# mataiyuan/ASD-SLAM

Measured on AMD Instinct MI355X. Metric: frames/sec end-to-end tracking+LocalBA, KITTI 00 mono @2000 keypoints, higher is better.
Workload: dtype f32

## Files before the change

asd-slam_amd/csrc/asdnet.hip:

```cpp
#include "ctx.h"

#include <algorithm>
#include <cmath>
#include <cstring>

typedef float f32x16 __attribute__((ext_vector_type(16)));
typedef float f32x4 __attribute__((ext_vector_type(4)));


namespace {

struct LayerSpec { int cout, cin, k, stride, pad; };
const LayerSpec kLayers[7] = {{32, 1, 3, 1, 1},   {32, 32, 3, 1, 1},   {64, 32, 3, 2, 1},  {64, 64, 3, 1, 1},
                              {128, 64, 3, 2, 1}, {128, 128, 3, 1, 1}, {128, 128, 8, 1, 0}};

template <int CIN, int COUT, int HIN, int S, int ROWS, int WM, int WN, int KC, int PP = 1, int RING = 2>
struct ConvCfg {
  static constexpr int HO = HIN / S;
  static constexpr int INROWS = (ROWS - 1) * S + 3;
  static constexpr int INCOLS = (HO - 1) * S + 3;
  static constexpr int CPAD = CIN + 4;
  static constexpr int NW = WM * WN;
  static constexpr int NTH = 64 * NW;
  static constexpr int M_PATCH = ROWS * HO;
  static constexpr int M_WG = PP * M_PATCH;
  static constexpr int MT = M_WG / 32 / WM;
  static constexpr int NT = COUT / 32 / WN;
  static constexpr int NCC = CIN / KC;
  static constexpr int NSTAGE = 9 * NCC;
  static constexpr int WCHUNK = KC * COUT;
  static constexpr int WQUADS = WCHUNK / 4;
  static constexpr int WREGS = (WQUADS + NTH - 1) / NTH;
  static constexpr int ACT_FLOATS = INROWS * INCOLS * CPAD;
  static constexpr int LDS_BYTES = (PP * ACT_FLOATS + RING * WCHUNK) * 4;
  static_assert(RING == 2 || RING == 3, "weight ring depth");
  static_assert(NW == 4 || NW == 8, "4 or 8 waves per workgroup");
  static_assert(M_WG % (32 * WM) == 0 && COUT % (32 * WN) == 0, "tile split");
  static_assert(WQUADS % NTH == 0 || WQUADS < NTH, "weight stage: whole float4 rounds per thread, or a single partial round");
  static_assert(HO % ROWS == 0 && CIN % KC == 0 && KC % 8 == 0, "shape");
  static_assert(PP == 1 || ROWS == HO, "several patches per workgroup only for whole-patch bands");
  static_assert(M_PATCH % 32 == 0, "32-pixel MFMA tiles must not straddle patches");
};

template <int CIN, int COUT, int HIN, int S, int ROWS, int WM, int WN, int KC, int PP = 1, int RING = 2, int ABL = 0, bool FUSE1 = false>
__global__ __launch_bounds__(64 * WM * WN) void k_conv_mfma(const void* __restrict__ in_, const float* __restrict__ wimg,
                                                           const float* __restrict__ bias, float* __restrict__ out,
                                                           const float* __restrict__ w1, const float* __restrict__ b1, int n) {
  using C = ConvCfg<CIN, COUT, HIN, S, ROWS, WM, WN, KC, PP, RING>;
  constexpr int NTH = C::NTH;
  extern __shared__ __attribute__((aligned(16))) float smem[];
  float* sact = smem;
  float* sw = smem + PP * C::ACT_FLOATS;
  const int t = threadIdx.x, lane = t & 63, wave = t >> 6;
  const int wm = wave / WN, wn = wave % WN;
  constexpr int BANDS = C::HO / ROWS;
  const int patch = (blockIdx.x / BANDS) * PP, band = blockIdx.x % BANDS;
  const int r0 = band * ROWS;

  if constexpr (FUSE1) {
    static_assert(!FUSE1 || (CIN == 32 && HIN == 32 && S == 1 && PP == 1), "conv1 fusion is for conv2 only");
    float* pin = sw + RING * C::WCHUNK;
    float* wsh = pin + (ROWS + 4) * 36;
    float* red = wsh + 320;
    const uint8_t* patches = static_cast<const uint8_t*>(in_);
    for (int i = t; i < (ROWS + 4) * 36; i += NTH) pin[i] = 0.f;
    for (int i = t; i < 288; i += NTH) wsh[i] = w1[i];
    if (t < 32) wsh[288 + t] = b1[t];
    const bool ld = C::NW == 4 || wave < 4;
    const uchar4 v = ld ? reinterpret_cast<const uchar4*>(patches + (size_t)patch * 1024)[t] : make_uchar4(0, 0, 0, 0);
    const float inv255 = (float)(1.0 / 255);
    float x[4] = {v.x * inv255, v.y * inv255, v.z * inv255, v.w * inv255};
#pragma unroll
    for (int k = 0; k < 4; ++k) asm volatile("" : "+v"(x[k]));
    float s = (x[0] + x[1]) + (x[2] + x[3]);
    for (int off = 32; off >= 1; off >>= 1) s += __shfl_xor(s, off);
    if (lane == 0 && ld) red[wave] = s;
    asd_syncthreads();
    const float mean = ((red[0] + red[1]) + (red[2] + red[3])) * (1.0f / 1024.0f);
    float d[4], ss = 0.f;
    for (int k = 0; k < 4; ++k) { d[k] = x[k] - mean; ss += d[k] * d[k]; }
    for (int off = 32; off >= 1; off >>= 1) ss += __shfl_xor(ss, off);
    if (lane == 0 && ld) red[4 + wave] = ss;
    asd_syncthreads();
    const float sd = sqrtf(((red[4] + red[5]) + (red[6] + red[7])) * (1.0f / 1023.0f)) + 1e-7f;
    if (ld) {
      const int idx = t * 4, y = idx >> 5, x0 = idx & 31;
      const int j = y - (r0 - 2);
      if (j >= 0 && j < ROWS + 4)
        for (int k = 0; k < 4; ++k) pin[j * 36 + x0 + k + 1] = d[k] / sd;
    }
    asd_syncthreads();
    constexpr int NPIX = C::INROWS * C::INCOLS;
    static_assert(NTH % 8 == 0, "a thread must keep its cout quad across items");
    if (!(ABL & 1)) {
      const int q = t & 7;
      float wq[4][9], bq[4];
#pragma unroll
      for (int c = 0; c < 4; ++c) {
        bq[c] = wsh[288 + 4 * q + c];
#pragma unroll
        for (int k = 0; k < 9; ++k) wq[c][k] = wsh[(4 * q + c) * 9 + k];
      }
      for (int item = t; item < NPIX * 8; item += NTH) {
        const int pix = item >> 3;
        const int i = pix % C::INCOLS, j = pix / C::INCOLS;
        const int oy = r0 - 1 + j, ox = i - 1;
        f32x4 r = {0.f, 0.f, 0.f, 0.f};
        if (oy >= 0 && oy < 32 && ox >= 0 && ox < 32) {
          float a[9];
#pragma unroll
          for (int ky = 0; ky < 3; ++ky)
#pragma unroll
            for (int kx = 0; kx < 3; ++kx) a[ky * 3 + kx] = pin[(j + ky) * 36 + ox + kx];
#pragma unroll
          for (int c = 0; c < 4; ++c) {
            float acc1 = bq[c];
#pragma unroll
            for (int k = 0; k < 9; ++k) acc1 += a[k] * wq[c][k];
            r[c] = acc1 > 0.f ? acc1 : 0.f;
          }
        }
        *reinterpret_cast<f32x4*>(sact + pix * C::CPAD + 4 * q) = r;
      }
    }
  } else {
    const float* inp = static_cast<const float*>(in_) + (size_t)patch * HIN * HIN * CIN;
    constexpr int C4 = CIN / 4;
    constexpr int NPIXB = C::INROWS * C::INCOLS;
    if (!(ABL & 1))
    for (int idx = t; idx < PP * NPIXB * C4; idx += NTH) {
      const int c4 = idx % C4, pixg = idx / C4;
      const int pp = pixg / NPIXB, pix = pixg % NPIXB;
      const int i = pix % C::INCOLS, j = pix / C::INCOLS;
      const int iy = r0 * S - 1 + j, ix = i - 1;
      f32x4 v = {0.f, 0.f, 0.f, 0.f};
      if (iy >= 0 && iy < HIN && ix >= 0 && ix < HIN && patch + pp < n)
        v = *reinterpret_cast<const f32x4*>(inp + (size_t)pp * HIN * HIN * CIN + ((size_t)iy * HIN + ix) * CIN + c4 * 4);
      *reinterpret_cast<f32x4*>(sact + pp * C::ACT_FLOATS + pix * C::CPAD + c4 * 4) = v;
    }
  }
  constexpr int NPRE = RING == 3 ? 2 : 1;
  for (int ps = 0; ps < NPRE && ps < C::NSTAGE; ++ps)
    for (int r = 0; r < C::WREGS; ++r)
      if (C::WQUADS >= NTH || t < C::WQUADS)
        *reinterpret_cast<f32x4*>(sw + ps * C::WCHUNK + (r * NTH + t) * 4) =
            *reinterpret_cast<const f32x4*>(wimg + (size_t)ps * C::WCHUNK + (r * NTH + t) * 4);
  asd_syncthreads();

  f32x16 acc[C::MT][C::NT];
  for (int mt = 0; mt < C::MT; ++mt)
    for (int nt = 0; nt < C::NT; ++nt)
      for (int r = 0; r < 16; ++r) acc[mt][nt][r] = 0.f;

  const int h = lane >> 5, li = lane & 31;
  int abase[C::MT];
  for (int mt = 0; mt < C::MT; ++mt) {
    const int m = (wm * C::MT + mt) * 32 + li;
    const int pp = PP > 1 ? m / C::M_PATCH : 0, mm = m - pp * C::M_PATCH;
    const int rr = mm / C::HO, ox = mm % C::HO;
    abase[mt] = pp * C::ACT_FLOATS + ((rr * S) * C::INCOLS + ox * S) * C::CPAD + 4 * h;
  }
  const int bbase = (h * COUT + wn * C::NT * 32 + li) * 4;
  constexpr int STEPS = KC / 8;

  auto load_ops = [&](int s, int c8, f32x4 (&a)[C::MT], f32x4 (&b)[C::NT]) {
    const int tap = s / C::NCC, cc = s % C::NCC;
    const int tapoff = ((tap / 3) * C::INCOLS + (tap % 3)) * C::CPAD + cc * KC;
    const float* swb = sw + (s % RING) * C::WCHUNK;
#pragma unroll
    for (int mt = 0; mt < C::MT; ++mt) a[mt] = *reinterpret_cast<const f32x4*>(sact + abase[mt] + tapoff + c8 * 8);
#pragma unroll
    for (int nt = 0; nt < C::NT; ++nt) b[nt] = *reinterpret_cast<const f32x4*>(swb + bbase + c8 * 2 * COUT * 4 + nt * 128);
  };
  auto mfma_step = [&](const f32x4 (&a)[C::MT], const f32x4 (&b)[C::NT]) {
#pragma unroll
    for (int jj = 0; jj < 4; ++jj)
#pragma unroll
      for (int mt = 0; mt < C::MT; ++mt)
#pragma unroll
        for (int nt = 0; nt < C::NT; ++nt)
          if (!(ABL & 2)) acc[mt][nt] = __builtin_amdgcn_mfma_f32_32x32x2f32(a[mt][jj], b[nt][jj], acc[mt][nt], 0, 0, 0);
          else { asm volatile("" :: "v"(a[mt][jj]), "v"(b[nt][jj])); }
  };

  if constexpr (RING == 3) {
    f32x4 a0[C::MT], b0[C::NT], a1[C::MT], b1[C::NT];
    load_ops(0, 0, a0, b0);
    for (int s = 0; s < C::NSTAGE; ++s) {
      f32x4 wreg[C::WREGS];
      const bool pre = s + 2 < C::NSTAGE && !(ABL & 16);
      if (pre) {
        const float* wsrc = wimg + (size_t)(s + 2) * C::WCHUNK;
        for (int r = 0; r < C::WREGS; ++r)
          if (C::WQUADS >= NTH || t < C::WQUADS) wreg[r] = *reinterpret_cast<const f32x4*>(wsrc + (r * NTH + t) * 4);
      }
#pragma unroll
      for (int c8 = 0; c8 < STEPS; c8 += 2) {
        if (c8 + 1 < STEPS) load_ops(s, c8 + 1, a1, b1);
        else if (s + 1 < C::NSTAGE) load_ops(s + 1, 0, a1, b1);
        mfma_step(a0, b0);
        if (c8 + 1 < STEPS) {
          if (c8 + 2 < STEPS) load_ops(s, c8 + 2, a0, b0);
          else if (s + 1 < C::NSTAGE) load_ops(s + 1, 0, a0, b0);
          mfma_step(a1, b1);
        } else {
#pragma unroll
          for (int mt = 0; mt < C::MT; ++mt) a0[mt] = a1[mt];
#pragma unroll
          for (int nt = 0; nt < C::NT; ++nt) b0[nt] = b1[nt];
        }
      }
      if (pre) {
        float* swn = sw + ((s + 2) % 3) * C::WCHUNK;
        for (int r = 0; r < C::WREGS; ++r)
          if (C::WQUADS >= NTH || t < C::WQUADS) *reinterpret_cast<f32x4*>(swn + (r * NTH + t) * 4) = wreg[r];
      }
      if (!(ABL & 8)) asd_syncthreads();
    }
  } else {
    for (int s = 0; s < C::NSTAGE; ++s) {
      f32x4 wreg[C::WREGS];
      if (s + 1 < C::NSTAGE && !(ABL & 16)) {
        const float* wsrc = wimg + (size_t)(s + 1) * C::WCHUNK;
        for (int r = 0; r < C::WREGS; ++r)
          if (C::WQUADS >= NTH || t < C::WQUADS) wreg[r] = *reinterpret_cast<const f32x4*>(wsrc + (r * NTH + t) * 4);
      }
#pragma unroll
      for (int c8 = 0; c8 < STEPS; ++c8) {
        f32x4 a[C::MT], b[C::NT];
        load_ops(s, c8, a, b);
        mfma_step(a, b);
      }
      if (s + 1 < C::NSTAGE && !(ABL & 16)) {
        float* swn = sw + ((s + 1) & 1) * C::WCHUNK;
        for (int r = 0; r < C::WREGS; ++r)
          if (C::WQUADS >= NTH || t < C::WQUADS) *reinterpret_cast<f32x4*>(swn + (r * NTH + t) * 4) = wreg[r];
      }
      if (!(ABL & 8)) asd_syncthreads();
    }
  }

  float* op = out + ((size_t)patch * C::HO + r0) * C::HO * COUT;
  for (int nt = 0; nt < C::NT; ++nt) {
    const int co = (wn * C::NT + nt) * 32 + li;
    const float bv = bias[co];
    for (int mt = 0; mt < C::MT; ++mt) {
      const int pp = PP > 1 ? ((wm * C::MT + mt) * 32) / C::M_PATCH : 0;
      if (PP > 1 && patch + pp >= n) continue;
      for (int r = 0; r < 16; ++r) {
        const int m = (wm * C::MT + mt) * 32 + (r & 3) + 8 * (r >> 2) + 4 * h;
        const size_t o = (size_t)pp * C::HO * C::HO * COUT + (size_t)(m - pp * C::M_PATCH) * COUT + co;
        float v = acc[mt][nt][r] + bv;
        if (!(ABL & 4)) op[o] = v > 0.f ? v : 0.f;
        else { asm volatile("" :: "v"(v)); }
      }
    }
  }
}

template <int CIN, int COUT, int HIN, int S, int ROWS, int WM, int WN, int KC>
__global__ __launch_bounds__(256) void k_conv_mfma_p(const float* __restrict__ in, const float* __restrict__ wimg,
                                                     const float* __restrict__ bias, float* __restrict__ out, int ntiles) {
  using C = ConvCfg<CIN, COUT, HIN, S, ROWS, WM, WN, KC>;
  static_assert(C::NSTAGE >= 2, "need two stages to hide the band prefetch");
  static_assert(C::NW == 4, "the persistent form is written for 4 waves");
  extern __shared__ __attribute__((aligned(16))) float smem[];
  float* sact0 = smem;
  float* sw = smem + 2 * C::ACT_FLOATS;
  const int t = threadIdx.x, lane = t & 63, wave = t >> 6;
  const int wm = wave / WN, wn = wave % WN;
  constexpr int BANDS = C::HO / ROWS;
  constexpr int C4 = CIN / 4;
  constexpr int NELEM = C::INROWS * C::INCOLS * C4;
  constexpr int NPREF = (NELEM + 255) / 256;
  int tile = blockIdx.x;
  if (tile >= ntiles) return;

  f32x4 pre[NPREF];
#define LOAD_TILE(TILE)                                                                           \
  {                                                                                               \
    const int patch_ = (TILE) / BANDS, r0_ = ((TILE) % BANDS) * ROWS;                             \
    const float* inp_ = in + (size_t)patch_ * HIN * HIN * CIN;                                    \
    _Pragma("unroll") for (int p = 0; p < NPREF; ++p) {                                           \
      const int idx = t + p * 256;                                                                \
      f32x4 v = {0.f, 0.f, 0.f, 0.f};                                                             \
      if (idx < NELEM) {                                                                          \
        const int c4 = idx % C4, pix = idx / C4;                                                  \
        const int i = pix % C::INCOLS, j = pix / C::INCOLS;                                       \
        const int iy = r0_ * S - 1 + j, ix = i - 1;                                               \
        if (iy >= 0 && iy < HIN && ix >= 0 && ix < HIN)                                           \
          v = *reinterpret_cast<const f32x4*>(inp_ + ((size_t)iy * HIN + ix) * CIN + c4 * 4);     \
      }                                                                                           \
      pre[p] = v;                                                                                 \
    }                                                                                             \
  }
#define STORE_TILE(DST)                                                                           \
  {                                                                                               \
    _Pragma("unroll") for (int p = 0; p < NPREF; ++p) {                                           \
      const int idx = t + p * 256;                                                                \
      if (idx < NELEM) {                                                                          \
        const int c4 = idx % C4, pix = idx / C4;                                                  \
        *reinterpret_cast<f32x4*>((DST) + pix * C::CPAD + c4 * 4) = pre[p];                       \
      }                                                                                           \
    }                                                                                             \
  }
  LOAD_TILE(tile);
  STORE_TILE(sact0);
  for (int r = 0; r < C::WREGS; ++r)
    *reinterpret_cast<f32x4*>(sw + (r * 256 + t) * 4) = *reinterpret_cast<const f32x4*>(wimg + (r * 256 + t) * 4);
  asd_syncthreads();

  const int h = lane >> 5, li = lane & 31;
  int abase[C::MT];
  for (int mt = 0; mt < C::MT; ++mt) {
    const int m = (wm * C::MT + mt) * 32 + li;
    const int rr = m / C::HO, ox = m % C::HO;
    abase[mt] = ((rr * S) * C::INCOLS + ox * S) * C::CPAD + 4 * h;
  }
  const int bbase = (h * COUT + wn * C::NT * 32 + li) * 4;
  float bv[C::NT];
  for (int nt = 0; nt < C::NT; ++nt) bv[nt] = bias[(wn * C::NT + nt) * 32 + li];

  int cur = 0, g = 0;
  while (true) {
    const int next = tile + gridDim.x;
    const bool has_next = next < ntiles;
    const float* sact = sact0 + cur * C::ACT_FLOATS;
    f32x16 acc[C::MT][C::NT];
    for (int mt = 0; mt < C::MT; ++mt)
      for (int nt = 0; nt < C::NT; ++nt)
        for (int r = 0; r < 16; ++r) acc[mt][nt][r] = 0.f;
    for (int s = 0; s < C::NSTAGE; ++s) {
      f32x4 wreg[C::WREGS];
      {
        const int sn = (s + 1 == C::NSTAGE) ? 0 : s + 1;
        const float* wsrc = wimg + (size_t)sn * C::WCHUNK;
        for (int r = 0; r < C::WREGS; ++r) wreg[r] = *reinterpret_cast<const f32x4*>(wsrc + (r * 256 + t) * 4);
      }
      if (s == 0 && has_next) LOAD_TILE(next);
      const int tap = s / C::NCC, cc = s % C::NCC;
      const int tapoff = ((tap / 3) * C::INCOLS + (tap % 3)) * C::CPAD + cc * KC;
      const float* swb = sw + (g & 1) * C::WCHUNK;
#pragma unroll
      for (int c8 = 0; c8 < KC / 8; ++c8) {
        f32x4 a[C::MT], b[C::NT];
#pragma unroll
        for (int mt = 0; mt < C::MT; ++mt) a[mt] = *reinterpret_cast<const f32x4*>(sact + abase[mt] + tapoff + c8 * 8);
#pragma unroll
        for (int nt = 0; nt < C::NT; ++nt)
          b[nt] = *reinterpret_cast<const f32x4*>(swb + bbase + c8 * 2 * COUT * 4 + nt * 128);
#pragma unroll
        for (int jj = 0; jj < 4; ++jj)
#pragma unroll
          for (int mt = 0; mt < C::MT; ++mt)
#pragma unroll
            for (int nt = 0; nt < C::NT; ++nt)
              acc[mt][nt] = __builtin_amdgcn_mfma_f32_32x32x2f32(a[mt][jj], b[nt][jj], acc[mt][nt], 0, 0, 0);
      }
      {
        float* swn = sw + ((g + 1) & 1) * C::WCHUNK;
        for (int r = 0; r < C::WREGS; ++r) *reinterpret_cast<f32x4*>(swn + (r * 256 + t) * 4) = wreg[r];
      }
      if (s == 1 && has_next) STORE_TILE(sact0 + (cur ^ 1) * C::ACT_FLOATS);
      asd_syncthreads();
      ++g;
    }
    {
      const int patch = tile / BANDS, r0 = (tile % BANDS) * ROWS;
      float* op = out + ((size_t)patch * C::HO + r0) * C::HO * COUT;
      for (int nt = 0; nt < C::NT; ++nt) {
        const int co = (wn * C::NT + nt) * 32 + li;
        for (int mt = 0; mt < C::MT; ++mt)
          for (int r = 0; r < 16; ++r) {
            const int m = (wm * C::MT + mt) * 32 + (r & 3) + 8 * (r >> 2) + 4 * h;
            const float v = acc[mt][nt][r] + bv[nt];
            op[(size_t)m * COUT + co] = v > 0.f ? v : 0.f;
          }
      }
    }
    if (!has_next) break;
    tile = next;
    cur ^= 1;
  }
#undef LOAD_TILE
#undef STORE_TILE
}

#ifndef ASD_X3_ABL
#define ASD_X3_ABL 0
#endif
#ifndef ASD_X3_S16
#define ASD_X3_S16 1
#endif
#define ASD_X3_PD 2
#ifndef ASD_X3_RB
#define ASD_X3_RB 3
#endif
typedef __bf16 bf16x8 __attribute__((ext_vector_type(8)));
typedef uint32_t u32x4 __attribute__((ext_vector_type(4)));

template <int CIN, int COUT, int HIN, int S, int ROWS, int WM, int WN, int PP = 1, int NP = 3>
struct X3Cfg {
  static constexpr int HO = HIN / S;
  static constexpr int INROWS = (ROWS - 1) * S + 3;
  static constexpr int INCOLS = (HO - 1) * S + 3;
  static constexpr int PIXB = CIN * 2 * NP + 16;
  static constexpr int GRPB = 16 * NP;
  static constexpr bool PLANAR = NP == 2 && S == 2 && ASD_X3_S16 != 0;
  static constexpr int GSTR = PLANAR ? 16 : GRPB;
  static constexpr int PSTR = PLANAR ? CIN * 2 : 16;
  static constexpr int NW = WM * WN;
  static constexpr int NTH = 64 * NW;
  static constexpr int M_PATCH = ROWS * HO;
  static constexpr int M_WG = PP * M_PATCH;
  static constexpr int MT = M_WG / 32 / WM;
  static constexpr int NT = COUT / 32 / WN;
  static constexpr int KCH = ASD_X3_S16 ? 32 : 16;
  static constexpr int NC16 = CIN / KCH;
  static constexpr int NCHUNK = 9 * NC16;
  static constexpr int CHUNKB = KCH * 2 * NP * COUT;
  static constexpr int ACT_BYTES = INROWS * INCOLS * PIXB;
  static constexpr int LDS_BYTES = PP * ACT_BYTES;
  static_assert((PIXB / 16) % 2 == 1, "pixel stride must be an odd multiple of 16 B");
  static constexpr int NCW = COUT / WN;
  static_assert(M_WG % (32 * WM) == 0 && COUT % WN == 0 && NCW % (ASD_X3_S16 ? 16 : 32) == 0 && CIN % KCH == 0 && HO % ROWS == 0, "tile split");
  static_assert(PP == 1 || ROWS == HO, "several patches per workgroup only for whole-patch bands");
  static_assert(M_PATCH % 32 == 0, "32-pixel MFMA tiles must not straddle patches");
};

__device__ inline void split8(const f32x4& v0, const f32x4& v1, u32x4& ph, u32x4& pm, u32x4& pl) {
  float x[8] = {v0[0], v0[1], v0[2], v0[3], v1[0], v1[1], v1[2], v1[3]};
  uint32_t hu[8], mu[8], lu[8];
#pragma unroll
  for (int j = 0; j < 8; ++j) {
    const uint32_t u = __float_as_uint(x[j]);
    const float r1 = x[j] - __uint_as_float(u & 0xffff0000u);
    const uint32_t r1u = __float_as_uint(r1);
    const float r2 = r1 - __uint_as_float(r1u & 0xffff0000u);
    hu[j] = u; mu[j] = r1u; lu[j] = __float_as_uint(r2);
  }
#pragma unroll
  for (int q = 0; q < 4; ++q) {
    ph[q] = __builtin_amdgcn_perm(hu[2 * q + 1], hu[2 * q], 0x07060302u);
    pm[q] = __builtin_amdgcn_perm(mu[2 * q + 1], mu[2 * q], 0x07060302u);
    pl[q] = __builtin_amdgcn_perm(lu[2 * q + 1], lu[2 * q], 0x07060302u);
  }
}


constexpr float kActScale = 16.f;

typedef _Float16 f16x8 __attribute__((ext_vector_type(8)));
__device__ inline void split8_f16(const f32x4& v0, const f32x4& v1, float scale, u32x4& ph, u32x4& pl) {
  float x[8] = {v0[0], v0[1], v0[2], v0[3], v1[0], v1[1], v1[2], v1[3]};
  f16x8 h, l;
#pragma unroll
  for (int j = 0; j < 8; ++j) {
    const float xs = x[j] * scale;
    h[j] = (_Float16)xs;
    l[j] = (_Float16)(xs - (float)h[j]);
  }
  ph = __builtin_bit_cast(u32x4, h);
  pl = __builtin_bit_cast(u32x4, l);
}

__device__ __forceinline__ void split4_mix(float x0, float x1, float x2, float x3, float s, uint32_t (&h)[2], uint32_t (&l)[2]) {
  asm("v_fma_mixlo_f16 %0, %8, %4, 0\n\t"
      "v_fma_mixlo_f16 %1, %8, %6, 0\n\t"
      "v_fma_mixhi_f16 %0, %8, %5, 0\n\t"
      "v_fma_mixhi_f16 %1, %8, %7, 0\n\t"
      "v_fma_mixlo_f16 %2, %8, %4, -%0 op_sel_hi:[0,0,1]\n\t"
      "v_fma_mixlo_f16 %3, %8, %6, -%1 op_sel_hi:[0,0,1]\n\t"
      "v_fma_mixhi_f16 %2, %8, %5, -%0 op_sel:[0,0,1] op_sel_hi:[0,0,1]\n\t"
      "v_fma_mixhi_f16 %3, %8, %7, -%1 op_sel:[0,0,1] op_sel_hi:[0,0,1]\n\t"
      "s_nop 0"
      : "=&v"(h[0]), "=&v"(h[1]), "=&v"(l[0]), "=&v"(l[1])
      : "v"(x0), "v"(x1), "v"(x2), "v"(x3), "s"(s));
}


__global__ __launch_bounds__(256) void k_patch_stats(const uint8_t* __restrict__ patches, float* __restrict__ stats, int n) {
  __shared__ float red[8];
  const int t = threadIdx.x, lane = t & 63, wave = t >> 6, patch = blockIdx.x;
  const uchar4 v = reinterpret_cast<const uchar4*>(patches + (size_t)patch * 1024)[t];
  const float inv255 = (float)(1.0 / 255);
  float x[4] = {v.x * inv255, v.y * inv255, v.z * inv255, v.w * inv255};
#pragma unroll
  for (int k = 0; k < 4; ++k) asm volatile("" : "+v"(x[k]));
  float sum = (x[0] + x[1]) + (x[2] + x[3]);
  for (int off = 32; off >= 1; off >>= 1) sum += __shfl_xor(sum, off);
  if (lane == 0) red[wave] = sum;
  asd_syncthreads();
  const float mean = ((red[0] + red[1]) + (red[2] + red[3])) * (1.0f / 1024.0f);
  float d[4], ss = 0.f;
  for (int k = 0; k < 4; ++k) { d[k] = x[k] - mean; ss += d[k] * d[k]; }
  for (int off = 32; off >= 1; off >>= 1) ss += __shfl_xor(ss, off);
  if (lane == 0) red[4 + wave] = ss;
  asd_syncthreads();
  const float sd = sqrtf(((red[4] + red[5]) + (red[6] + red[7])) * (1.0f / 1023.0f)) + 1e-7f;
  if (t == 0) { stats[2 * (size_t)patch] = mean; stats[2 * (size_t)patch + 1] = sd; }
}

template <int CIN, int COUT, int HIN, int S, int ROWS, int WM, int WN, int PP, bool FUSE1 = false, int NP = 3, bool PAIR = false>
__device__ __forceinline__ void conv_x3_tile(const int bid, const void* __restrict__ in_, const uint8_t* __restrict__ wimg,
                                                         const float* __restrict__ bias, float* __restrict__ out,
                                                         const float* __restrict__ w1, const float* __restrict__ b1, int n,
                                                         unsigned long long* __restrict__ stamps, float in_scale, float out_scale,
                                                         const float* __restrict__ stats = nullptr) {
  using C = X3Cfg<CIN, COUT, HIN, S, ROWS, WM, WN, PP, NP>;
  constexpr int NTH = C::NTH, MT = C::MT, NCW = C::NCW;
  static_assert(!PAIR || (NP == 2 && ASD_X3_S16), "the pair format belongs to the two-piece form on the 16x16x32 shape");
  extern __shared__ __attribute__((aligned(16))) uint8_t smem_b[];
  int t = threadIdx.x;
  asm volatile("" : "+v"(t));
  const int lane = t & 63, wave = t >> 6;
  const int wm = wave / WN, wn = wave % WN;
  const int h = lane >> 5, li = lane & 31;
  constexpr int BANDS = C::HO / ROWS;
  const int patch = (bid / BANDS) * PP, band = bid % BANDS;
  const int r0 = band * ROWS;
  unsigned long long st_t0 = 0, st_t1 = 0;
  if (stamps) st_t0 = st_t1 = __builtin_amdgcn_s_memtime();
#define X3_STAMP(k) do { if (stamps && t == 0) stamps[16 * bid + (k)] = __builtin_amdgcn_s_memtime() - st_t0; } while (0)

  constexpr bool S16 = ASD_X3_S16;
  constexpr int SUB = S16 ? 2 : 1, KG = C::KCH / 8, TW = 32 / SUB;
  const int kg = S16 ? lane >> 4 : h, lr = S16 ? lane & 15 : li;
  const uint8_t* wl = wimg + ((size_t)kg * COUT + wn * NCW + lr) * 16;
  constexpr int NB = NCW / TW;
  auto load_b = [&](int c, u32x4 (&b)[NB][NP]) {
    const uint8_t* wc = wl + (size_t)((ASD_X3_ABL & 1) ? (c & 1) : c) * C::CHUNKB;
#pragma unroll
    for (int nb = 0; nb < NB; ++nb)
#pragma unroll
      for (int p = 0; p < NP; ++p) b[nb][p] = *reinterpret_cast<const u32x4*>(wc + (size_t)p * KG * COUT * 16 + nb * TW * 16);
  };
  constexpr int RB = C::NCHUNK % ASD_X3_RB == 0 ? ASD_X3_RB : 3;
  static_assert(C::NCHUNK % RB == 0, "chunk count");
  u32x4 br[RB][NB][NP];
#pragma unroll
  for (int d = 0; d < RB - 1; ++d) load_b(d, br[d]);

  if constexpr (FUSE1) {
    static_assert(!FUSE1 || (CIN == 32 && HIN == 32 && S == 1 && PP == 1 && (C::NW == 4 || C::NW == 8)), "conv1 fusion is for conv2 only");
    float* pin = reinterpret_cast<float*>(smem_b + C::ACT_BYTES);
    float* wsh = pin + (ROWS + 4) * 36;
    float* red = wsh + 320;
    const uint8_t* patches = static_cast<const uint8_t*>(in_);
    for (int i = t; i < (ROWS + 4) * 36; i += NTH) {
      const int j = i / 36, c = i % 36, y = r0 - 2 + j;
      if (!(c >= 1 && c <= 32 && y >= 0 && y < 32)) pin[i] = 0.f;
    }
    for (int i = t; i < 288; i += NTH) wsh[i] = w1[i];
    if (t < 32) wsh[288 + t] = b1[t];
    const bool ld = C::NW == 4 || wave < 4;
    const uchar4 v = ld ? reinterpret_cast<const uchar4*>(patches + (size_t)patch * 1024)[t] : make_uchar4(0, 0, 0, 0);
    const float inv255 = (float)(1.0 / 255);
    float x[4] = {v.x * inv255, v.y * inv255, v.z * inv255, v.w * inv255};
#pragma unroll
    for (int k = 0; k < 4; ++k) asm volatile("" : "+v"(x[k]));
    float d[4], sd;
    if (stats) {
      const float mean = stats[2 * (size_t)patch];
      sd = stats[2 * (size_t)patch + 1];
      for (int k = 0; k < 4; ++k) d[k] = x[k] - mean;
      X3_STAMP(9);
    } else {
      float sum = (x[0] + x[1]) + (x[2] + x[3]);
      for (int off = 32; off >= 1; off >>= 1) sum += __shfl_xor(sum, off);
      X3_STAMP(9);
      if (lane == 0 && ld) red[wave] = sum;
      asd_syncthreads();
      const float mean = ((red[0] + red[1]) + (red[2] + red[3])) * (1.0f / 1024.0f);
      float ss = 0.f;
      for (int k = 0; k < 4; ++k) { d[k] = x[k] - mean; ss += d[k] * d[k]; }
      for (int off = 32; off >= 1; off >>= 1) ss += __shfl_xor(ss, off);
      if (lane == 0 && ld) red[4 + wave] = ss;
      asd_syncthreads();
      sd = sqrtf(((red[4] + red[5]) + (red[6] + red[7])) * (1.0f / 1023.0f)) + 1e-7f;
    }
    if (ld) {
      const int idx = t * 4, y = idx >> 5, x0 = idx & 31;
      const int j = y - (r0 - 2);
      if (j >= 0 && j < ROWS + 4)
        for (int k = 0; k < 4; ++k) pin[j * 36 + x0 + k + 1] = d[k] / sd;
    }
    asd_syncthreads();
    if (stamps) st_t1 = __builtin_amdgcn_s_memtime();
    constexpr int NPIX = C::INROWS * C::INCOLS;
    if (!(ASD_X3_ABL & 2)) {
      const int q = t & 3;
      float wq[8][9], bq1[8];
#pragma unroll
      for (int c = 0; c < 8; ++c) {
        bq1[c] = wsh[288 + 8 * q + c];
#pragma unroll
        for (int k = 0; k < 9; ++k) wq[c][k] = wsh[(8 * q + c) * 9 + k];
      }
      for (int item = t; item < NPIX * 4; item += NTH) {
        const int pix = item >> 2;
        const int i = pix % C::INCOLS, j = pix / C::INCOLS;
        const int oy = r0 - 1 + j, ox = i - 1;
        f32x4 ra = {0.f, 0.f, 0.f, 0.f}, rb = {0.f, 0.f, 0.f, 0.f};
        if (oy >= 0 && oy < 32 && ox >= 0 && ox < 32) {
          float a[9];
#pragma unroll
          for (int ky = 0; ky < 3; ++ky)
#pragma unroll
            for (int kx = 0; kx < 3; ++kx) a[ky * 3 + kx] = pin[(j + ky) * 36 + ox + kx];
#pragma unroll
          for (int c = 0; c < 8; ++c) {
            float acc1 = bq1[c];
#pragma unroll
            for (int k = 0; k < ((ASD_X3_ABL & 32) ? 1 : 9); ++k) acc1 += a[k] * wq[c][k];
            const float r = acc1 > 0.f ? acc1 : 0.f;
            if (c < 4) ra[c] = r; else rb[c - 4] = r;
          }
        }
        u32x4 ph, pm, pl;
        uint8_t* dst = smem_b + pix * C::PIXB + q * C::GSTR;
        if constexpr (NP == 2) {
          split8_f16(ra, rb, in_scale, ph, pl);
          *reinterpret_cast<u32x4*>(dst) = ph;
          *reinterpret_cast<u32x4*>(dst + C::PSTR) = pl;
        } else {
          if constexpr ((ASD_X3_ABL & 64) != 0) { ph = __builtin_bit_cast(u32x4, ra); pm = __builtin_bit_cast(u32x4, rb); pl = ph; }
          else split8(ra, rb, ph, pm, pl);
          *reinterpret_cast<u32x4*>(dst) = ph;
          *reinterpret_cast<u32x4*>(dst + 16) = pm;
          *reinterpret_cast<u32x4*>(dst + 32) = pl;
        }
      }
    }
  } else if constexpr (PAIR) {
    const uint8_t* inb = static_cast<const uint8_t*>(in_) + (size_t)patch * HIN * HIN * CIN * 4;
    constexpr int C8 = CIN / 8;
    constexpr int NPIXB = C::INROWS * C::INCOLS;
    static_assert(NTH % C8 == 0, "a thread keeps its channel group");
    constexpr int PSTEP = NTH / C8;
    constexpr int NROUND = (PP * NPIXB + PSTEP - 1) / PSTEP;
    constexpr int SBATCH = 8;
    const int c8 = t % C8, pix0 = t / C8;
    for (int rb = 0; rb < ((ASD_X3_ABL & 2) ? 0 : NROUND); rb += SBATCH) {
      u32x4 v0[SBATCH], v1[SBATCH];
#pragma unroll
      for (int b = 0; b < SBATCH; ++b) {
        const int pixg = pix0 + (rb + b) * PSTEP;
        const int pp = pixg / NPIXB, pix = pixg % NPIXB;
        const int i = pix % C::INCOLS, j = pix / C::INCOLS;
        const int iy = r0 * S - 1 + j, ix = i - 1;
        v0[b] = u32x4{0, 0, 0, 0}; v1[b] = u32x4{0, 0, 0, 0};
        if (rb + b < NROUND && pixg < PP * NPIXB && iy >= 0 && iy < HIN && ix >= 0 && ix < HIN && patch + pp < n) {
          const uint8_t* src = inb + ((size_t)pp * HIN * HIN * CIN + ((size_t)iy * HIN + ix) * CIN + c8 * 8) * 4;
          v0[b] = *reinterpret_cast<const u32x4*>(src);
          v1[b] = *reinterpret_cast<const u32x4*>(src + 16);
        }
      }
#pragma unroll
      for (int b = 0; b < SBATCH; ++b) {
        const int pixg = pix0 + (rb + b) * PSTEP;
        if (rb + b < NROUND && pixg < PP * NPIXB) {
          uint8_t* dst = smem_b + (pixg / NPIXB) * C::ACT_BYTES + (pixg % NPIXB) * C::PIXB + c8 * C::GSTR;
          *reinterpret_cast<u32x4*>(dst) = v0[b];
          *reinterpret_cast<u32x4*>(dst + C::PSTR) = v1[b];
        }
      }
    }
  } else
  {
    const float* inp = static_cast<const float*>(in_) + (size_t)patch * HIN * HIN * CIN;
    constexpr int C8 = CIN / 8;
    constexpr int NPIXB = C::INROWS * C::INCOLS;
    static_assert(NTH % C8 == 0, "a thread keeps its cin group");
    constexpr int PSTEP = NTH / C8;
    constexpr int NROUND = (PP * NPIXB + PSTEP - 1) / PSTEP;
    constexpr int SBATCH = 8;
    const int c8 = t % C8, pix0 = t / C8;
    for (int rb = 0; rb < ((ASD_X3_ABL & 2) ? 0 : NROUND); rb += SBATCH) {
      f32x4 v0[SBATCH], v1[SBATCH];
#pragma unroll
      for (int b = 0; b < SBATCH; ++b) {
        const int pixg = pix0 + (rb + b) * PSTEP;
        const int pp = pixg / NPIXB, pix = pixg % NPIXB;
        const int i = pix % C::INCOLS, j = pix / C::INCOLS;
        const int iy = r0 * S - 1 + j, ix = i - 1;
        v0[b] = f32x4{0.f, 0.f, 0.f, 0.f}; v1[b] = f32x4{0.f, 0.f, 0.f, 0.f};
        if (rb + b < NROUND && pixg < PP * NPIXB && iy >= 0 && iy < HIN && ix >= 0 && ix < HIN && patch + pp < n) {
          const float* src = inp + (size_t)pp * HIN * HIN * CIN + ((size_t)iy * HIN + ix) * CIN + c8 * 8;
          v0[b] = *reinterpret_cast<const f32x4*>(src);
          v1[b] = *reinterpret_cast<const f32x4*>(src + 4);
        }
      }
#pragma unroll
      for (int b = 0; b < SBATCH; ++b) {
        const int pixg = pix0 + (rb + b) * PSTEP;
        if (rb + b < NROUND && pixg < PP * NPIXB) {
          u32x4 ph, pm, pl;
          uint8_t* dst = smem_b + (pixg / NPIXB) * C::ACT_BYTES + (pixg % NPIXB) * C::PIXB + c8 * C::GSTR;
          if constexpr (NP == 2) {
            split8_f16(v0[b], v1[b], in_scale, ph, pl);
            *reinterpret_cast<u32x4*>(dst) = ph;
            *reinterpret_cast<u32x4*>(dst + C::PSTR) = pl;
          } else {
            split8(v0[b], v1[b], ph, pm, pl);
            *reinterpret_cast<u32x4*>(dst) = ph;
            *reinterpret_cast<u32x4*>(dst + 16) = pm;
            *reinterpret_cast<u32x4*>(dst + 32) = pl;
          }
        }
      }
    }
  }
  X3_STAMP(12);
  asd_syncthreads();
  X3_STAMP(13);

  constexpr int NA = MT * SUB, AR = S16 ? 4 : 16;
  typedef float accv __attribute__((ext_vector_type(S16 ? 4 : 16)));
  accv acc[NA][NB];
  for (int ma = 0; ma < NA; ++ma)
    for (int nb = 0; nb < NB; ++nb)
      for (int r = 0; r < AR; ++r) acc[ma][nb][r] = 0.f;
  auto tile_pixel = [&](int sg, int r16) -> int {
    if constexpr (NP == 2 && S16) {
      if constexpr (S == 1 && C::HO >= 16) return sg * 16 + (r16 < 4 ? 2 * r16 : r16 < 12 ? 2 * r16 - 7 : 2 * r16 - 16);
      else if constexpr (S == 2 && C::HO >= 16) return sg * 16 + r16;
      else if constexpr (S == 2) return sg * 16 + (r16 < 4 ? r16 : r16 < 12 ? r16 + 4 : r16 - 8);
      else {
        static_assert(S == 2 || C::HO >= 16 || (PP == 1 && C::HO == 8 && ROWS == 8), "eight rows x two columns per sub-tile");
        const int j = r16 < 4 ? r16 : r16 < 12 ? r16 - 4 : r16 - 8;
        return j * C::HO + 2 * sg + (r16 >= 4 && r16 < 12 ? 1 : 0);
      }
    } else return sg * TW + r16;
  };
  int abase[NA];
  for (int ma = 0; ma < NA; ++ma) {
    const int m = tile_pixel((wm * MT * 32 + ma * TW) / TW, lr);
    const int pp = PP > 1 ? m / C::M_PATCH : 0, mm = m - pp * C::M_PATCH;
    const int rr = mm / C::HO, ox = mm % C::HO;
    abase[ma] = pp * C::ACT_BYTES + ((rr * S) * C::INCOLS + ox * S) * C::PIXB + kg * C::GSTR;
  }
  auto chunk_off = [&](int c) {
    const int tap = c / C::NC16, c16 = c % C::NC16;
    return ((tap / 3) * C::INCOLS + (tap % 3)) * C::PIXB + c16 * (KG * C::GSTR);
  };
  auto load_a = [&](int off, u32x4 (&a)[NP]) {
#pragma unroll
    for (int p = 0; p < NP; ++p) a[p] = *reinterpret_cast<const u32x4*>(smem_b + off + p * C::PSTR);
  };
  auto bf = [](const u32x4& v) { return __builtin_bit_cast(bf16x8, v); };
  auto hf = [](const u32x4& v) { return __builtin_bit_cast(f16x8, v); };
  auto mma = [&](const u32x4& x, const u32x4& y, accv& c) {
    if constexpr ((ASD_X3_ABL & 8) != 0) { asm volatile("" ::"v"(x), "v"(y)); }
#ifdef ASD_PAIR_NOTRANS
    else if constexpr (PAIR) c = __builtin_amdgcn_mfma_f32_16x16x32_f16(hf(x), hf(y), c, 0, 0, 0);
#endif
    else if constexpr (PAIR) c = __builtin_amdgcn_mfma_f32_16x16x32_f16(hf(y), hf(x), c, 0, 0, 0);
    else if constexpr (NP == 2 && S16) c = __builtin_amdgcn_mfma_f32_16x16x32_f16(hf(x), hf(y), c, 0, 0, 0);
    else if constexpr (NP == 2) c = __builtin_amdgcn_mfma_f32_32x32x16_f16(hf(x), hf(y), c, 0, 0, 0);
    else if constexpr (S16) c = __builtin_amdgcn_mfma_f32_16x16x32_bf16(bf(x), bf(y), c, 0, 0, 0);
    else c = __builtin_amdgcn_mfma_f32_32x32x16_bf16(bf(x), bf(y), c, 0, 0, 0);
  };

  constexpr int PD = ASD_X3_PD, RS = PD + 1;
  static_assert((RB * NA) % RS == 0, "ring slots must be static");
  u32x4 ar[RS][NP];
#pragma unroll
  for (int q = 0; q < PD; ++q) load_a(abase[q % NA] + chunk_off(q / NA), ar[q]);
  unsigned long long st_c = 0, st_r = 0;
  if (stamps) { st_c = __builtin_amdgcn_s_memtime(); st_r = __builtin_amdgcn_s_memrealtime(); }
  for (int c0 = 0; c0 < C::NCHUNK; c0 += RB) {
    int offs[RB + PD / NA + 2];
#pragma unroll
    for (int u = 0; u < RB + PD / NA + 2; ++u) offs[u] = chunk_off(c0 + u < C::NCHUNK ? c0 + u : C::NCHUNK - 1);
#pragma unroll
    for (int u = 0; u < RB; ++u) {
      const int c = c0 + u;
      load_b(c + RB - 1 < C::NCHUNK ? c + RB - 1 : C::NCHUNK - 1, br[(u + RB - 1) % RB]);
      __builtin_amdgcn_sched_group_barrier(0x020, NP * NB, 0);
      const u32x4 (&bc)[NB][NP] = br[u];
#pragma unroll
      for (int ma = 0; ma < NA; ++ma) {
        const int q = u * NA + ma;
        const int qn = q + PD;
        load_a(abase[qn % NA] + offs[qn / NA], ar[qn % RS]);
        const u32x4 (&ac)[NP] = ar[q % RS];
#pragma unroll
        for (int nb = 0; nb < NB; ++nb) {
          if constexpr (NP == 2) {
            mma(ac[1], bc[nb][0], acc[ma][nb]);
            mma(ac[0], bc[nb][1], acc[ma][nb]);
            mma(ac[0], bc[nb][0], acc[ma][nb]);
          } else {
            mma(ac[2], bc[nb][0], acc[ma][nb]);
            mma(ac[0], bc[nb][2], acc[ma][nb]);
            mma(ac[1], bc[nb][1], acc[ma][nb]);
            mma(ac[1], bc[nb][0], acc[ma][nb]);
            mma(ac[0], bc[nb][1], acc[ma][nb]);
            mma(ac[0], bc[nb][0], acc[ma][nb]);
          }
        }
#pragma unroll
        for (int p = 0; p < NP; ++p) {
          __builtin_amdgcn_sched_group_barrier(0x008, (NP * (NP + 1) / 2) * NB / NP, 0);
          __builtin_amdgcn_sched_group_barrier(0x100, 1, 0);
        }
      }
    }
  }

  if (stamps) {
    asm volatile("s_nop 0" ::"v"(acc[NA - 1][NB - 1][0]));
    const unsigned long long e_c = __builtin_amdgcn_s_memtime(), e_r = __builtin_amdgcn_s_memrealtime();
    if (t == 0) { stamps[16 * bid] = e_c - st_c; stamps[16 * bid + 1] = e_r - st_r; stamps[16 * bid + 2] = st_t1 - st_t0; stamps[16 * bid + 3] = st_c - st_t1; stamps[16 * bid + 6] = st_t0; }
  }
  if constexpr (PAIR) {
    uint8_t* opb = reinterpret_cast<uint8_t*>(out) + ((size_t)patch * C::HO + r0) * C::HO * COUT * 4;
    for (int nb = 0; nb < NB; ++nb) {
      const int co0 = wn * NCW + nb * TW + 4 * kg;
      const f32x4 bv = *reinterpret_cast<const f32x4*>(bias + co0);
      for (int ma = 0; ma < NA; ++ma) {
        const int m0 = wm * MT * 32 + ma * TW;
        const int pp = PP > 1 ? m0 / C::M_PATCH : 0;
        if (PP > 1 && patch + pp >= n) continue;
        const int m = tile_pixel(m0 / TW, lr);
        float v[4];
#pragma unroll
        for (int r = 0; r < 4; ++r) { const float x = acc[ma][nb][r] * out_scale + bv[r]; v[r] = x < 0.f ? 0.f : x; }
        uint32_t hh[2], ll[2];
        split4_mix(v[0], v[1], v[2], v[3], kActScale, hh, ll);
        const auto s0 = __builtin_amdgcn_permlane16_swap(hh[0], ll[0], false, false);
        const auto s1 = __builtin_amdgcn_permlane16_swap(hh[1], ll[1], false, false);
        uint8_t* o = opb + ((size_t)pp * C::HO * C::HO + (size_t)(m - pp * C::M_PATCH)) * COUT * 4 + (co0 >> 3) * 32 + (kg & 1) * 16;
        if (!(ASD_X3_ABL & 4) || hh[0] == 0x12345u) *reinterpret_cast<u32x4*>(o) = u32x4{s0[0], s1[0], s0[1], s1[1]};
      }
    }
  } else {
  float* op = out + ((size_t)patch * C::HO + r0) * C::HO * COUT;
  for (int nb = 0; nb < NB; ++nb) {
    const int co = wn * NCW + nb * TW + lr;
    const float bv = bias[co];
    for (int ma = 0; ma < NA; ++ma) {
      const int m0 = wm * MT * 32 + ma * TW;
      const int pp = PP > 1 ? m0 / C::M_PATCH : 0;
      if (PP > 1 && patch + pp >= n) continue;
      for (int r = 0; r < AR; ++r) {
        const int m = S16 ? tile_pixel(m0 / TW, 4 * kg + r) : m0 + (r & 3) + 8 * (r >> 2) + 4 * h;
        const size_t o = (size_t)pp * C::HO * C::HO * COUT + (size_t)(m - pp * C::M_PATCH) * COUT + co;
        const float v = (NP == 2 ? acc[ma][nb][r] * out_scale : acc[ma][nb][r]) + bv;
        if (!(ASD_X3_ABL & 4) || v == 12345.f) op[o] = NP == 2 ? (v < 0.f ? 0.f : v) : (v > 0.f ? v : 0.f);
      }
    }
  }
  }
  if (stamps && t == 0) { const unsigned long long e = __builtin_amdgcn_s_memtime(); stamps[16 * bid + 5] = e - st_t0; stamps[16 * bid + 7] = e; }
}

#ifndef ASD_L2_MINWG
#define ASD_L2_MINWG 3
#endif
template <int CIN, int COUT, int HIN, int S, int ROWS, int WM, int WN, int PP, bool FUSE1 = false, int NP = 3, bool PAIR = false>
__global__ __launch_bounds__(64 * WM * WN, (FUSE1 && NP == 2) ? ASD_L2_MINWG : 1) void k_conv_x3(const void* __restrict__ in_, const uint8_t* __restrict__ wimg,
                                                         const float* __restrict__ bias, float* __restrict__ out,
                                                         const float* __restrict__ w1, const float* __restrict__ b1, int n,
                                                         unsigned long long* __restrict__ stamps, float in_scale, float out_scale,
                                                         const float* __restrict__ stats) {
  const int bid = (S == 2 && CIN == 32) ? (int)(gridDim.x - 1 - blockIdx.x) : (int)blockIdx.x;
  conv_x3_tile<CIN, COUT, HIN, S, ROWS, WM, WN, PP, FUSE1, NP, PAIR>(bid, in_, wimg, bias, out, w1, b1, n, stamps, in_scale, out_scale, stats);
}

constexpr int FC_SK = 16;
constexpr int FC_KCH = 128;
constexpr int FC_MT = 1;
__global__ __launch_bounds__(256) void k_fc_mfma(const float* __restrict__ act, const float* __restrict__ wimg,
                                                 float* __restrict__ part, int n, int npad) {
  __shared__ __attribute__((aligned(16))) float sa[FC_MT * 32 * (FC_KCH + 4)];
  const int t = threadIdx.x, lane = t & 63, wave = t >> 6;
  const int h = lane >> 5, li = lane & 31;
  const int p0 = blockIdx.x * 32 * FC_MT, sk = blockIdx.y;
  constexpr int KPER = 8192 / FC_SK;
  f32x16 acc[FC_MT];
  for (int m = 0; m < FC_MT; ++m)
    for (int r = 0; r < 16; ++r) acc[m][r] = 0.f;
  for (int st = 0; st < KPER / FC_KCH; ++st) {
    const int k0 = sk * KPER + st * FC_KCH;
    asd_syncthreads();
    for (int idx = t; idx < FC_MT * 32 * (FC_KCH / 4); idx += 256) {
      const int c4 = idx % (FC_KCH / 4), row = idx / (FC_KCH / 4);
      int p = p0 + row;
      if (p >= n) p = n - 1;
      *reinterpret_cast<f32x4*>(sa + row * (FC_KCH + 4) + c4 * 4) =
          *reinterpret_cast<const f32x4*>(act + (size_t)p * 8192 + k0 + c4 * 4);
    }
    asd_syncthreads();
    const float* wb = wimg + ((size_t)(k0 / 8) * 2 + h) * 128 * 4 + (wave * 32 + li) * 4;
#pragma unroll 4
    for (int c8 = 0; c8 < FC_KCH / 8; ++c8) {
      const f32x4 b = *reinterpret_cast<const f32x4*>(wb + (size_t)c8 * 2 * 128 * 4);
      f32x4 a[FC_MT];
#pragma unroll
      for (int m = 0; m < FC_MT; ++m) a[m] = *reinterpret_cast<const f32x4*>(sa + (m * 32 + li) * (FC_KCH + 4) + c8 * 8 + 4 * h);
#pragma unroll
      for (int jj = 0; jj < 4; ++jj)
#pragma unroll
        for (int m = 0; m < FC_MT; ++m) acc[m] = __builtin_amdgcn_mfma_f32_32x32x2f32(a[m][jj], b[jj], acc[m], 0, 0, 0);
    }
  }
  for (int m = 0; m < FC_MT; ++m) {
    if (p0 + m * 32 >= npad) break;
    float* op = part + ((size_t)sk * npad + p0 + m * 32) * 128;
    for (int r = 0; r < 16; ++r) {
      const int row = (r & 3) + 8 * (r >> 2) + 4 * h;
      op[(size_t)row * 128 + wave * 32 + li] = acc[m][r];
    }
  }
}

constexpr int FCS_MP = 64;
constexpr int FCS_SLAB = 128;
constexpr int FCS_ROWB = FCS_SLAB * 6 + 16;
__global__ __launch_bounds__(256) void k_fc_x3(const float* __restrict__ act, const uint8_t* __restrict__ wimg,
                                               float* __restrict__ part, int n, int npad) {
  __shared__ __attribute__((aligned(16))) uint8_t sa[FCS_MP * FCS_ROWB];
  typedef float f4 __attribute__((ext_vector_type(4)));
  const int t = threadIdx.x, lane = t & 63, wave = t >> 6;
  const int kg = lane >> 4, lr = lane & 15;
  const int p0 = blockIdx.x * FCS_MP, sk = blockIdx.y;
  constexpr int KPER = 8192 / FC_SK, NSLAB = KPER / FCS_SLAB, NCH = KPER / 32;
  static_assert(KPER % FCS_SLAB == 0 && NCH >= 3, "split-K slice");
  constexpr int CHUNKB = 32 * 6 * 128;
  const uint8_t* wl = wimg + (size_t)(sk * (KPER / 32)) * CHUNKB + ((size_t)kg * 128 + wave * 32 + lr) * 16;
  auto load_b = [&](int c, u32x4 (&b)[2][3]) {
    const uint8_t* wc = wl + (size_t)c * CHUNKB;
#pragma unroll
    for (int nb = 0; nb < 2; ++nb)
#pragma unroll
      for (int p = 0; p < 3; ++p) b[nb][p] = *reinterpret_cast<const u32x4*>(wc + (size_t)p * 4 * 128 * 16 + nb * 256);
  };
  auto bf = [](const u32x4& v) { return __builtin_bit_cast(bf16x8, v); };
  u32x4 br[3][2][3];
  load_b(0, br[0]);
  load_b(1, br[1]);
  f4 acc[4][2];
  for (int ma = 0; ma < 4; ++ma)
    for (int nb = 0; nb < 2; ++nb)
      for (int r = 0; r < 4; ++r) acc[ma][nb][r] = 0.f;
  int c = 0;
  for (int slab = 0; slab < NSLAB; ++slab) {
    const int k0 = sk * KPER + slab * FCS_SLAB;
    asd_syncthreads();
    {
      f32x4 v0[4], v1[4];
#pragma unroll
      for (int i = 0; i < 4; ++i) {
        const int item = t + i * 256, row = item >> 4, g = item & 15;
        int p = p0 + row;
        if (p >= n) p = n - 1;
        const float* src = act + (size_t)p * 8192 + k0 + g * 8;
        v0[i] = *reinterpret_cast<const f32x4*>(src);
        v1[i] = *reinterpret_cast<const f32x4*>(src + 4);
      }
#pragma unroll
      for (int i = 0; i < 4; ++i) {
        const int item = t + i * 256, row = item >> 4, g = item & 15;
        u32x4 ph, pm, pl;
        split8(v0[i], v1[i], ph, pm, pl);
        uint8_t* dst = sa + row * FCS_ROWB + g * 48;
        *reinterpret_cast<u32x4*>(dst) = ph;
        *reinterpret_cast<u32x4*>(dst + 16) = pm;
        *reinterpret_cast<u32x4*>(dst + 32) = pl;
      }
    }
    asd_syncthreads();
#pragma unroll
    for (int cs = 0; cs < FCS_SLAB / 32; ++cs, ++c) {
      auto step = [&](u32x4 (&bc)[2][3], u32x4 (&bn)[2][3]) {
        load_b(c + 2 < NCH ? c + 2 : NCH - 1, bn);
#pragma unroll
        for (int ma = 0; ma < 4; ++ma) {
          u32x4 a[3];
          const uint8_t* ap = sa + (ma * 16 + lr) * FCS_ROWB + (cs * 4 + kg) * 48;
#pragma unroll
          for (int p = 0; p < 3; ++p) a[p] = *reinterpret_cast<const u32x4*>(ap + p * 16);
#pragma unroll
          for (int nb = 0; nb < 2; ++nb) {
            acc[ma][nb] = __builtin_amdgcn_mfma_f32_16x16x32_bf16(bf(a[2]), bf(bc[nb][0]), acc[ma][nb], 0, 0, 0);
            acc[ma][nb] = __builtin_amdgcn_mfma_f32_16x16x32_bf16(bf(a[0]), bf(bc[nb][2]), acc[ma][nb], 0, 0, 0);
            acc[ma][nb] = __builtin_amdgcn_mfma_f32_16x16x32_bf16(bf(a[1]), bf(bc[nb][1]), acc[ma][nb], 0, 0, 0);
            acc[ma][nb] = __builtin_amdgcn_mfma_f32_16x16x32_bf16(bf(a[1]), bf(bc[nb][0]), acc[ma][nb], 0, 0, 0);
            acc[ma][nb] = __builtin_amdgcn_mfma_f32_16x16x32_bf16(bf(a[0]), bf(bc[nb][1]), acc[ma][nb], 0, 0, 0);
            acc[ma][nb] = __builtin_amdgcn_mfma_f32_16x16x32_bf16(bf(a[0]), bf(bc[nb][0]), acc[ma][nb], 0, 0, 0);
          }
        }
      };
      const int slot = c % 3;
      if (slot == 0) step(br[0], br[2]);
      else if (slot == 1) step(br[1], br[0]);
      else step(br[2], br[1]);
    }
  }
  if (p0 >= npad) return;
  float* op = part + ((size_t)sk * npad + p0) * 128;
  for (int ma = 0; ma < 4; ++ma)
    for (int nb = 0; nb < 2; ++nb)
      for (int r = 0; r < 4; ++r) {
        const int row = ma * 16 + 4 * kg + r;
        if (p0 + row < npad) op[(size_t)row * 128 + wave * 32 + nb * 16 + lr] = acc[ma][nb][r];
      }
}

constexpr int FCP_ROWB = FCS_SLAB * 4 + 16;
__global__ __launch_bounds__(256) void k_fc_x2(const uint8_t* __restrict__ act, const uint8_t* __restrict__ wimg,
                                               float* __restrict__ part, int n, int npad, float out_scale) {
  __shared__ __attribute__((aligned(16))) uint8_t sa[FCS_MP * FCP_ROWB];
  typedef float f4 __attribute__((ext_vector_type(4)));
  const int t = threadIdx.x, lane = t & 63, wave = t >> 6;
  const int kg = lane >> 4, lr = lane & 15;
  const int p0 = blockIdx.x * FCS_MP, sk = blockIdx.y;
  constexpr int KPER = 8192 / FC_SK, NSLAB = KPER / FCS_SLAB, NCH = KPER / 32;
  constexpr int CHUNKB = 32 * 4 * 128;
  const uint8_t* wl = wimg + (size_t)(sk * (KPER / 32)) * CHUNKB + ((size_t)kg * 128 + wave * 32 + lr) * 16;
  auto load_b = [&](int c, u32x4 (&b)[2][2]) {
    const uint8_t* wc = wl + (size_t)c * CHUNKB;
#pragma unroll
    for (int nb = 0; nb < 2; ++nb)
#pragma unroll
      for (int p = 0; p < 2; ++p) b[nb][p] = *reinterpret_cast<const u32x4*>(wc + (size_t)p * 4 * 128 * 16 + nb * 256);
  };
  auto hf = [](const u32x4& v) { return __builtin_bit_cast(f16x8, v); };
  u32x4 br[3][2][2];
  load_b(0, br[0]);
  load_b(1, br[1]);
  f4 acc[4][2];
  for (int ma = 0; ma < 4; ++ma)
    for (int nb = 0; nb < 2; ++nb)
      for (int r = 0; r < 4; ++r) acc[ma][nb][r] = 0.f;
  int c = 0;
  for (int slab = 0; slab < NSLAB; ++slab) {
    const int k0 = sk * KPER + slab * FCS_SLAB;
    asd_syncthreads();
    {
      u32x4 v0[4], v1[4];
#pragma unroll
      for (int i = 0; i < 4; ++i) {
        const int item = t + i * 256, row = item >> 4, g = item & 15;
        int p = p0 + row;
        if (p >= n) p = n - 1;
        const uint8_t* src = act + (size_t)p * 32768 + (size_t)(k0 / 8 + g) * 32;
        v0[i] = *reinterpret_cast<const u32x4*>(src);
        v1[i] = *reinterpret_cast<const u32x4*>(src + 16);
      }
#pragma unroll
      for (int i = 0; i < 4; ++i) {
        const int item = t + i * 256, row = item >> 4, g = item & 15;
        uint8_t* dst = sa + row * FCP_ROWB + g * 32;
        *reinterpret_cast<u32x4*>(dst) = v0[i];
        *reinterpret_cast<u32x4*>(dst + 16) = v1[i];
      }
    }
    asd_syncthreads();
#pragma unroll
    for (int cs = 0; cs < FCS_SLAB / 32; ++cs, ++c) {
      auto step = [&](u32x4 (&bc)[2][2], u32x4 (&bn)[2][2]) {
        load_b(c + 2 < NCH ? c + 2 : NCH - 1, bn);
#pragma unroll
        for (int ma = 0; ma < 4; ++ma) {
          const uint8_t* ap = sa + (ma * 16 + lr) * FCP_ROWB + (cs * 4 + kg) * 32;
          const u32x4 ah = *reinterpret_cast<const u32x4*>(ap), al = *reinterpret_cast<const u32x4*>(ap + 16);
#pragma unroll
          for (int nb = 0; nb < 2; ++nb) {
            acc[ma][nb] = __builtin_amdgcn_mfma_f32_16x16x32_f16(hf(al), hf(bc[nb][0]), acc[ma][nb], 0, 0, 0);
            acc[ma][nb] = __builtin_amdgcn_mfma_f32_16x16x32_f16(hf(ah), hf(bc[nb][1]), acc[ma][nb], 0, 0, 0);
            acc[ma][nb] = __builtin_amdgcn_mfma_f32_16x16x32_f16(hf(ah), hf(bc[nb][0]), acc[ma][nb], 0, 0, 0);
          }
        }
      };
      const int slot = c % 3;
      if (slot == 0) step(br[0], br[2]);
      else if (slot == 1) step(br[1], br[0]);
      else step(br[2], br[1]);
    }
  }
  if (p0 >= npad) return;
  float* op = part + ((size_t)sk * npad + p0) * 128;
  for (int ma = 0; ma < 4; ++ma)
    for (int nb = 0; nb < 2; ++nb)
      for (int r = 0; r < 4; ++r) {
        const int row = ma * 16 + 4 * kg + r;
        if (p0 + row < npad) op[(size_t)row * 128 + wave * 32 + nb * 16 + lr] = acc[ma][nb][r] * out_scale;
      }
}

__global__ __launch_bounds__(256) void k_absmax(const float* __restrict__ p, size_t n, unsigned* __restrict__ out) {
  unsigned m = 0;
  for (size_t i = (size_t)blockIdx.x * 256 + threadIdx.x; i < n; i += (size_t)gridDim.x * 256) m = max(m, __float_as_uint(p[i]) & 0x7fffffffu);
  for (int off = 32; off >= 1; off >>= 1) m = max(m, (unsigned)__shfl_xor((int)m, off));
  if ((threadIdx.x & 63) == 0 && m) atomicMax(out, m);
}

__global__ __launch_bounds__(256) void k_l2norm(const float* __restrict__ part, const float* __restrict__ bias,
                                                float* __restrict__ desc, int n, int npad, int* __restrict__ range_flag) {
  const int lane = threadIdx.x & 63, p = blockIdx.x * 4 + (threadIdx.x >> 6);
  if (p >= n) return;
  float v0 = 0.f, v1 = 0.f;
  for (int sk = 0; sk < FC_SK; ++sk) {
    v0 += part[((size_t)sk * npad + p) * 128 + lane];
    v1 += part[((size_t)sk * npad + p) * 128 + lane + 64];
  }
  v0 += bias[lane];
  v1 += bias[lane + 64];
  float ss = v0 * v0 + v1 * v1;
  for (int off = 32; off >= 1; off >>= 1) ss += __shfl_xor(ss, off);
  const float norm = sqrtf(ss + 1e-10f);
  if (range_flag && lane == 0 && !(fabsf(ss) <= 3.0e38f)) *range_flag = 1;
  desc[(size_t)p * 128 + lane] = v0 / norm;
  desc[(size_t)p * 128 + lane + 64] = v1 / norm;
}

constexpr bool kPairOK = ASD_X3_S16 != 0;
#define L2_CFG 32, 32, 32, 1, 4, 4, 1, 16, 1, 3
#define L3_CFG 32, 64, 32, 2, 4, 2, 2, 16
#define L4_CFG 64, 64, 16, 1, 8, 4, 1, 32, 1, 2
#define L5_CFG 64, 128, 16, 2, 4, 1, 4, 16, 1, 3
#define L6_CFG 128, 128, 8, 1, 8, 2, 2, 16, 1, 3
#ifndef ASD_L2_WMN
#define ASD_L2_WMN 4, 1
#endif
#ifndef ASD_L3_WMN
#if ASD_X3_S16
#define ASD_L3_WMN 1, 4
#else
#define ASD_L3_WMN 2, 2
#endif
#endif
#ifndef ASD_L4_WMN
#define ASD_L4_WMN 2, 2
#endif
#define L2S_CFG 32, 32, 32, 1, 8, ASD_L2_WMN, 1
#ifndef ASD_L3_ROWS
#define ASD_L3_ROWS 4
#endif
#define L3S_CFG 32, 64, 32, 2, ASD_L3_ROWS, ASD_L3_WMN, 1
#define L4S_CFG 64, 64, 16, 1, 8, ASD_L4_WMN, 1
#ifndef ASD_L5_RWMN
#if ASD_X3_S16
#define ASD_L5_RWMN 8, 1, 4
#else
#define ASD_L5_RWMN 4, 1, 4
#endif
#endif
#ifndef ASD_L6_WMN
#define ASD_L6_WMN 1, 4
#endif
#define L5S_CFG 64, 128, 16, 2, ASD_L5_RWMN, 1
#define L6S_CFG 128, 128, 8, 1, 8, ASD_L6_WMN, 1

template <int CIN, int COUT, int HIN, int S, int ROWS, int WM, int WN, int KC, int PP = 1, int RING = 2, bool FUSE1 = false>
hipError_t launch_conv(hipStream_t st, const void* in, const float* wimg, const float* bias, float* out, int n,
                       const float* w1 = nullptr, const float* b1 = nullptr) {
  using C = ConvCfg<CIN, COUT, HIN, S, ROWS, WM, WN, KC, PP, RING>;
  auto kern = k_conv_mfma<CIN, COUT, HIN, S, ROWS, WM, WN, KC, PP, RING, 0, FUSE1>;
  constexpr int lds = C::LDS_BYTES + (FUSE1 ? ((ROWS + 4) * 36 + 320 + 8) * 4 : 0);
  static_assert(lds <= 160 * 1024, "band + weight ring do not fit LDS");
  static AsdPerDeviceOnce attr_set;
  int dev_ = 0;
  (void)hipGetDevice(&dev_);
  if (attr_set.need(dev_)) {
    hipError_t e = hipFuncSetAttribute(reinterpret_cast<const void*>(kern), hipFuncAttributeMaxDynamicSharedMemorySize, lds);
    if (e != hipSuccess) return e;
    attr_set.done(dev_);
  }
  hipLaunchKernelGGL(kern, dim3(((n + PP - 1) / PP) * (C::HO / ROWS)), dim3(C::NTH), lds, st, in, wimg, bias, out, w1, b1, n);
  return hipGetLastError();
}

template <int CIN, int COUT, int HIN, int S, int ROWS, int WM, int WN, int KC>
hipError_t launch_conv_p(hipStream_t st, const float* in, const float* wimg, const float* bias, float* out, int n, int num_cu) {
  using C = ConvCfg<CIN, COUT, HIN, S, ROWS, WM, WN, KC>;
  auto kern = k_conv_mfma_p<CIN, COUT, HIN, S, ROWS, WM, WN, KC>;
  constexpr int lds = (2 * C::ACT_FLOATS + 2 * C::WCHUNK) * 4;
  static_assert(lds <= 160 * 1024, "double-buffered band does not fit LDS");
  static AsdPerDeviceOnce attr_set;
  int dev_ = 0;
  (void)hipGetDevice(&dev_);
  if (attr_set.need(dev_)) {
    hipError_t e = hipFuncSetAttribute(reinterpret_cast<const void*>(kern), hipFuncAttributeMaxDynamicSharedMemorySize, lds);
    if (e != hipSuccess) return e;
    attr_set.done(dev_);
  }
  const int ntiles = n * (C::HO / ROWS);
  const int per_cu = std::max(1, std::min(4, (160 * 1024) / lds));
  const int grid = std::min(ntiles, num_cu * per_cu);
  hipLaunchKernelGGL(kern, dim3(grid), dim3(256), lds, st, in, wimg, bias, out, ntiles);
  return hipGetLastError();
}

template <int CIN, int COUT, int HIN, int S, int ROWS, int WM, int WN, int PP, bool FUSE1 = false, int NP = 3, bool PAIR = false>
hipError_t launch_conv_x3(hipStream_t st, const void* in, const void* wimg, const float* bias, float* out, int n,
                          const float* w1 = nullptr, const float* b1 = nullptr, unsigned long long* stamps = nullptr, int* grid_out = nullptr,
                          float in_scale = 1.f, float out_scale = 1.f, const float* stats = nullptr) {
  using C = X3Cfg<CIN, COUT, HIN, S, ROWS, WM, WN, PP, NP>;
  auto kern = k_conv_x3<CIN, COUT, HIN, S, ROWS, WM, WN, PP, FUSE1, NP, PAIR>;
  constexpr int lds0 = C::LDS_BYTES + (FUSE1 ? ((ROWS + 4) * 36 + 320 + 8) * 4 : 0);
  static_assert(lds0 <= 160 * 1024, "band does not fit LDS");
  const int lds = lds0;
  static AsdPerDeviceOnce attr_set;
  int dev_ = 0;
  (void)hipGetDevice(&dev_);
  if (attr_set.need(dev_)) {
    hipError_t e = hipFuncSetAttribute(reinterpret_cast<const void*>(kern), hipFuncAttributeMaxDynamicSharedMemorySize, lds);
    if (e != hipSuccess) return e;
    attr_set.done(dev_);
  }
  const int ntiles = ((n + PP - 1) / PP) * (C::HO / ROWS);
  if (grid_out) *grid_out = ntiles;
  hipLaunchKernelGGL(kern, dim3(ntiles), dim3(C::NTH), lds, st, in, static_cast<const uint8_t*>(wimg), bias, out, w1, b1, n, stamps,
                     in_scale, out_scale, stats);
  return hipGetLastError();
}

inline void split3_host(float x, uint16_t& h, uint16_t& m, uint16_t& l) {
  uint32_t u, r1u, r2u;
  memcpy(&u, &x, 4);
  const uint32_t hu = u & 0xffff0000u;
  float hf; memcpy(&hf, &hu, 4);
  const float r1 = x - hf;
  memcpy(&r1u, &r1, 4);
  const uint32_t mu = r1u & 0xffff0000u;
  float mf; memcpy(&mf, &mu, 4);
  const float r2 = r1 - mf;
  memcpy(&r2u, &r2, 4);
  h = (uint16_t)(hu >> 16); m = (uint16_t)(mu >> 16); l = (uint16_t)(r2u >> 16);
}

inline void split2_host(float xs, uint16_t& h, uint16_t& l) {
  const _Float16 hh = (_Float16)xs;
  const _Float16 ll = (_Float16)(xs - (float)hh);
  memcpy(&h, &hh, 2);
  memcpy(&l, &ll, 2);
}

inline float weight_scale_f16(const float* w, size_t count, const std::vector<float>& inv, size_t per_cout) {
  float mx = 0.f;
  for (size_t i = 0; i < count; ++i) mx = std::max(mx, std::fabs(w[i] * inv[i / per_cout]));
  if (!(mx > 0.f) || !std::isfinite(mx)) return 1.f;
  int e;
  (void)std::frexp(mx, &e);
  return std::ldexp(1.f, 14 - e);
}

void build_wx3(const LayerSpec& L, const float* w, const std::vector<float>& inv, std::vector<uint16_t>& img, int np = 3, float wscale = 1.f) {
  img.assign((size_t)9 * L.cin * L.cout * np, 0);
  constexpr int kch = ASD_X3_S16 ? 32 : 16, kg = kch / 8;
  const int nc16 = L.cin / kch;
  for (int tap = 0; tap < 9; ++tap)
    for (int ci = 0; ci < L.cin; ++ci)
      for (int co = 0; co < L.cout; ++co) {
        const float v = w[((size_t)co * L.cin + ci) * 9 + tap] * inv[co];
        uint16_t p[3];
        if (np == 3) split3_host(v, p[0], p[1], p[2]);
        else split2_host(v * wscale, p[0], p[1]);
        const int c16 = ci / kch, hh = (ci % kch) / 8, j = ci % 8;
        for (int q = 0; q < np; ++q)
          img[(((((size_t)tap * nc16 + c16) * np + q) * kg + hh) * L.cout + co) * 8 + j] = p[q];
      }
}

void build_wimg(const LayerSpec& L, const float* w, const std::vector<float>& inv, std::vector<float>& img) {
  img.assign((size_t)9 * L.cin * L.cout, 0.f);
  for (int tap = 0; tap < 9; ++tap)
    for (int ci = 0; ci < L.cin; ++ci)
      for (int co = 0; co < L.cout; ++co) {
        const int c8 = ci / 8, hh = (ci % 8) / 4, jj = ci % 4;
        const size_t dst = ((((size_t)tap * (L.cin / 8) + c8) * 2 + hh) * L.cout + co) * 4 + jj;
        img[dst] = w[((size_t)co * L.cin + ci) * 9 + tap] * inv[co];
      }
}

}

int asdnet_alloc(asd_ctx* ctx) {
  const size_t np = (size_t)ctx->cfg.max_patches;
  const size_t npad = (np + 31) / 32 * 32;
  ASD_HIP_CHECK(ctx, hipMalloc(&ctx->d_act[0], np * 32768 * sizeof(float)));
  ASD_HIP_CHECK(ctx, hipMalloc(&ctx->d_act[1], np * 32768 * sizeof(float)));
  ASD_HIP_CHECK(ctx, hipMalloc(&ctx->d_part, (size_t)FC_SK * npad * 128 * sizeof(float)));
  ASD_HIP_CHECK(ctx, hipMalloc(&ctx->d_patches, np * 1024));
  ASD_HIP_CHECK(ctx, hipMalloc(&ctx->d_desc, np * 128 * sizeof(float)));
  ASD_HIP_CHECK(ctx, hipHostMalloc(reinterpret_cast<void**>(&ctx->h_range), 64));
  *ctx->h_range = 0;
  if (const char* e = getenv("ASD_ASDNET_PAIR")) ctx->net_pair = atoi(e) != 0;
  if (const char* e = getenv("ASD_ASDNET_RING")) ctx->ring_mask = atoi(e);
  return ASD_OK;
}

void asdnet_free(asd_ctx* ctx) {
  for (int i = 0; i < 2; ++i) if (ctx->d_act[i]) (void)hipFree(ctx->d_act[i]);
  if (ctx->d_part) (void)hipFree(ctx->d_part);
  if (ctx->d_patches) (void)hipFree(ctx->d_patches);
  if (ctx->d_desc) (void)hipFree(ctx->d_desc);
  if (ctx->h_range) (void)hipHostFree(ctx->h_range);
  if (ctx->d_w1) (void)hipFree(ctx->d_w1);
  for (int i = 0; i < 7; ++i) {
    if (ctx->d_bias[i]) (void)hipFree(ctx->d_bias[i]);
    if (ctx->d_wimg[i]) (void)hipFree(ctx->d_wimg[i]);
    if (ctx->d_wx3[i]) (void)hipFree(ctx->d_wx3[i]);
    if (ctx->d_wx2[i]) (void)hipFree(ctx->d_wx2[i]);
  }
}

static int asdnet_calibrate(asd_ctx* ctx, const float* const conv_w[7], const float* const bn_mean[7], const float* const bn_var[7], float eps);

int asdnet_load_weights(asd_ctx* ctx, const float* const conv_w[7], const float* const bn_mean[7],
                        const float* const bn_var[7], float eps) {
  for (int l = 0; l < 7; ++l) {
    const LayerSpec& L = kLayers[l];
    std::vector<float> inv(L.cout), bias(L.cout);
    for (int c = 0; c < L.cout; ++c) {
      inv[c] = 1.0f / std::sqrt(bn_var[l][c] + eps);
      bias[c] = -bn_mean[l][c] * inv[c];
    }
    if (!ctx->d_bias[l]) ASD_HIP_CHECK(ctx, hipMalloc(&ctx->d_bias[l], L.cout * sizeof(float)));
    ASD_HIP_CHECK(ctx, hipMemcpy(ctx->d_bias[l], bias.data(), L.cout * sizeof(float), hipMemcpyHostToDevice));
    std::vector<float> img;
    if (l == 0) {
      img.resize(32 * 9);
      for (int co = 0; co < 32; ++co)
        for (int k = 0; k < 9; ++k) img[co * 9 + k] = conv_w[0][co * 9 + k] * inv[co];
      if (!ctx->d_w1) ASD_HIP_CHECK(ctx, hipMalloc(&ctx->d_w1, img.size() * sizeof(float)));
      ASD_HIP_CHECK(ctx, hipMemcpy(ctx->d_w1, img.data(), img.size() * sizeof(float), hipMemcpyHostToDevice));
      continue;
    }
    if (l < 6) {
      build_wimg(L, conv_w[l], inv, img);
    } else {
      img.assign((size_t)8192 * 128, 0.f);
      for (int px = 0; px < 64; ++px)
        for (int c = 0; c < 128; ++c)
          for (int co = 0; co < 128; ++co) {
            const int k = px * 128 + c, k8 = k / 8, hh = (k % 8) / 4, jj = k % 4;
            img[(((size_t)k8 * 2 + hh) * 128 + co) * 4 + jj] = conv_w[6][((size_t)co * 128 + c) * 64 + px] * inv[co];
          }
    }
    if (!ctx->d_wimg[l]) ASD_HIP_CHECK(ctx, hipMalloc(&ctx->d_wimg[l], img.size() * sizeof(float)));
    ASD_HIP_CHECK(ctx, hipMemcpy(ctx->d_wimg[l], img.data(), img.size() * sizeof(float), hipMemcpyHostToDevice));
    if (l == 6) {
      std::vector<uint16_t> x3((size_t)8192 * 128 * 3, 0);
      for (int px = 0; px < 64; ++px)
        for (int c = 0; c < 128; ++c)
          for (int co = 0; co < 128; ++co) {
            const int k = px * 128 + c, c32 = k / 32, g = (k % 32) / 8, j = k % 8;
            uint16_t pc[3];
            split3_host(conv_w[6][((size_t)co * 128 + c) * 64 + px] * inv[co], pc[0], pc[1], pc[2]);
            for (int q = 0; q < 3; ++q) x3[((((size_t)c32 * 3 + q) * 4 + g) * 128 + co) * 8 + j] = pc[q];
          }
      if (!ctx->d_wx3[l]) ASD_HIP_CHECK(ctx, hipMalloc(&ctx->d_wx3[l], x3.size() * sizeof(uint16_t)));
      ASD_HIP_CHECK(ctx, hipMemcpy(ctx->d_wx3[l], x3.data(), x3.size() * sizeof(uint16_t), hipMemcpyHostToDevice));
      const float ws = weight_scale_f16(conv_w[6], (size_t)128 * 128 * 64, inv, (size_t)128 * 64);
      ctx->wx2_scale[l] = ws;
      std::vector<uint16_t> x2((size_t)8192 * 128 * 2, 0);
      for (int px = 0; px < 64; ++px)
        for (int c = 0; c < 128; ++c)
          for (int co = 0; co < 128; ++co) {
            const int k = px * 128 + c, c32 = k / 32, g = (k % 32) / 8, j = k % 8;
            uint16_t pc[2];
            split2_host(conv_w[6][((size_t)co * 128 + c) * 64 + px] * inv[co] * ws, pc[0], pc[1]);
            for (int q = 0; q < 2; ++q) x2[((((size_t)c32 * 2 + q) * 4 + g) * 128 + co) * 8 + j] = pc[q];
          }
      if (!ctx->d_wx2[l]) ASD_HIP_CHECK(ctx, hipMalloc(&ctx->d_wx2[l], x2.size() * sizeof(uint16_t)));
      ASD_HIP_CHECK(ctx, hipMemcpy(ctx->d_wx2[l], x2.data(), x2.size() * sizeof(uint16_t), hipMemcpyHostToDevice));
    }
    if (l < 6) {
      std::vector<uint16_t> x3;
      build_wx3(L, conv_w[l], inv, x3);
      if (!ctx->d_wx3[l]) ASD_HIP_CHECK(ctx, hipMalloc(&ctx->d_wx3[l], x3.size() * sizeof(uint16_t)));
      ASD_HIP_CHECK(ctx, hipMemcpy(ctx->d_wx3[l], x3.data(), x3.size() * sizeof(uint16_t), hipMemcpyHostToDevice));
      const float ws = weight_scale_f16(conv_w[l], (size_t)L.cout * L.cin * 9, inv, (size_t)L.cin * 9);
      ctx->wx2_scale[l] = ws;
      build_wx3(L, conv_w[l], inv, x3, 2, ws);
      if (!ctx->d_wx2[l]) ASD_HIP_CHECK(ctx, hipMalloc(&ctx->d_wx2[l], x3.size() * sizeof(uint16_t)));
      ASD_HIP_CHECK(ctx, hipMemcpy(ctx->d_wx2[l], x3.data(), x3.size() * sizeof(uint16_t), hipMemcpyHostToDevice));
    }
  }
  ctx->weights_loaded = true;
  return asdnet_calibrate(ctx, conv_w, bn_mean, bn_var, eps);
}

int asdnet_profile_collect_set(asd_ctx* ctx, int set);

static int asdnet_forward_one(asd_ctx* ctx, const uint8_t* d_patches, int n, float* d_desc, hipStream_t st, int* range_flag);
int asdnet_forward_device(asd_ctx* ctx, const uint8_t* d_patches, int n, float* d_desc, hipStream_t st, int* range_flag) {
  if (!ctx->weights_loaded) { ctx->set_error("asd_load_weights has not been called"); return ASD_ERR_NO_WEIGHTS; }
  if (n < 0 || n > ctx->cfg.max_patches) { ctx->set_error("n=%d exceeds max_patches=%d", n, ctx->cfg.max_patches); return ASD_ERR_CAPACITY; }
  if (n == 0) return ASD_OK;
  if (!st) st = ctx->stream;
  std::lock_guard<std::mutex> prof_lock(ctx->prof_mutex);
  return asdnet_forward_one(ctx, d_patches, n, d_desc, st, range_flag);
}
static int asdnet_forward_one(asd_ctx* ctx, const uint8_t* d_patches, int n, float* d_desc, hipStream_t st, int* range_flag) {
  float *a0 = ctx->d_act[0], *a1 = ctx->d_act[1];
  const int npad = (n + 31) / 32 * 32;
  const bool prof = ctx->prof_on;
  const int pset = ctx->prof_cur;
  if (prof && ctx->prof_pending[pset]) { int rc = asdnet_profile_collect_set(ctx, pset); if (rc != ASD_OK) return rc; }
#define PROF_MARK(i) do { if (prof) ASD_HIP_CHECK(ctx, hipEventRecord(ctx->prof_ev[pset][i], st)); } while (0)
  PROF_MARK(0);
  PROF_MARK(1);
  const bool p2 = ctx->net_pieces == 2;
  const bool pair = kPairOK && p2 && (ctx->net_split & 63) == 63 && ctx->net_pair && !ctx->d_calib;
  const float* x3_stats = nullptr;
#define X3_LAUNCH(CFG, FUSE, l, src, dst, w1p, b1p)                                                                                       \
  (pair ? launch_conv_x3<CFG, FUSE, 2, kPairOK>(st, src, ctx->d_wx2[l], ctx->d_bias[l], dst, n, w1p, b1p, nullptr, nullptr, kActScale,       \
                                     1.f / (kActScale * ctx->wx2_scale[l]), x3_stats)                                                               \
   : p2 ? launch_conv_x3<CFG, FUSE, 2>(st, src, ctx->d_wx2[l], ctx->d_bias[l], dst, n, w1p, b1p, nullptr, nullptr, kActScale,               \
                                     1.f / (kActScale * ctx->wx2_scale[l]), x3_stats)                                                               \
      : launch_conv_x3<CFG, FUSE, 3>(st, src, ctx->d_wx3[l], ctx->d_bias[l], dst, n, w1p, b1p, nullptr, nullptr, 1.f, 1.f,                \
                                     x3_stats))
  if (ctx->net_split & 1) {
    hipLaunchKernelGGL(k_patch_stats, dim3(n), dim3(256), 0, st, d_patches, ctx->d_part, n);
    ASD_HIP_CHECK(ctx, hipGetLastError());
    x3_stats = ctx->d_part;
    ASD_HIP_CHECK(ctx, (X3_LAUNCH(L2S_CFG, true, 1, d_patches, a1, ctx->d_w1, ctx->d_bias[0])));
    x3_stats = nullptr;
  }
  else ASD_HIP_CHECK(ctx, (launch_conv<L2_CFG, true>(st, d_patches, ctx->d_wimg[1], ctx->d_bias[1], a1, n, ctx->d_w1, ctx->d_bias[0])));
#define CALIB(l, buf, elems) do { if (ctx->d_calib) { hipLaunchKernelGGL(k_absmax, dim3(256), dim3(256), 0, st, buf, (size_t)n * (elems), ctx->d_calib + (l)); ASD_HIP_CHECK(ctx, hipGetLastError()); } } while (0)
  CALIB(1, a1, 32 * 32 * 32);
  PROF_MARK(2);
  if (ctx->net_split & 2) ASD_HIP_CHECK(ctx, (X3_LAUNCH(L3S_CFG, false, 2, a1, a0, nullptr, nullptr)));
  else
  ASD_HIP_CHECK(ctx, (launch_conv_p<L3_CFG>(st, a1, ctx->d_wimg[2], ctx->d_bias[2], a0, n, ctx->num_cu)));
  CALIB(2, a0, 16 * 16 * 64);
  PROF_MARK(3);
  const int ring = pair ? ctx->ring_mask : 0;
  float *src6 = a0, *dst6 = a1;
  if (ring & 4) {
    PROF_MARK(4);
    { const int rc = asdnet_ring_conv45(ctx, a0, a1, n, st); if (rc != ASD_OK) return rc; }
    src6 = a1; dst6 = a0;
  } else {
    if (ring & 1) { const int rc = asdnet_ring_conv(ctx, 3, a0, a1, n, st); if (rc != ASD_OK) return rc; }
    else if (ctx->net_split & 4) ASD_HIP_CHECK(ctx, (X3_LAUNCH(L4S_CFG, false, 3, a0, a1, nullptr, nullptr)));
    else ASD_HIP_CHECK(ctx, (launch_conv<L4_CFG>(st, a0, ctx->d_wimg[3], ctx->d_bias[3], a1, n)));
    CALIB(3, a1, 16 * 16 * 64);
    PROF_MARK(4);
    if (ctx->net_split & 8) ASD_HIP_CHECK(ctx, (X3_LAUNCH(L5S_CFG, false, 4, a1, a0, nullptr, nullptr)));
    else
    ASD_HIP_CHECK(ctx, (launch_conv<L5_CFG>(st, a1, ctx->d_wimg[4], ctx->d_bias[4], a0, n)));
  }
  CALIB(4, src6, 8 * 8 * 128);
  PROF_MARK(5);
  if (ring & 2) { const int rc = asdnet_ring_conv(ctx, 5, src6, dst6, n, st); if (rc != ASD_OK) return rc; }
  else if (ctx->net_split & 16) ASD_HIP_CHECK(ctx, (X3_LAUNCH(L6S_CFG, false, 5, src6, dst6, nullptr, nullptr)));
  else ASD_HIP_CHECK(ctx, (launch_conv<L6_CFG>(st, src6, ctx->d_wimg[5], ctx->d_bias[5], dst6, n)));
#undef X3_LAUNCH
  CALIB(5, dst6, 8 * 8 * 128);
#undef CALIB
  PROF_MARK(6);
  a1 = dst6;
  ctx->d_act6 = dst6;
  if (pair)
    hipLaunchKernelGGL(k_fc_x2, dim3((npad + FCS_MP - 1) / FCS_MP, FC_SK), dim3(256), 0, st, reinterpret_cast<const uint8_t*>(a1),
                       static_cast<const uint8_t*>(ctx->d_wx2[6]), ctx->d_part, n, npad, 1.f / (kActScale * ctx->wx2_scale[6]));
  else if (ctx->net_split & 32)
    hipLaunchKernelGGL(k_fc_x3, dim3((npad + FCS_MP - 1) / FCS_MP, FC_SK), dim3(256), 0, st, a1, static_cast<const uint8_t*>(ctx->d_wx3[6]), ctx->d_part, n, npad);
  else
    hipLaunchKernelGGL(k_fc_mfma, dim3((npad / 32 + FC_MT - 1) / FC_MT, FC_SK), dim3(256), 0, st, a1, ctx->d_wimg[6], ctx->d_part, n, npad);
  ASD_HIP_CHECK(ctx, hipGetLastError());
  PROF_MARK(7);
  hipLaunchKernelGGL(k_l2norm, dim3((n + 3) / 4), dim3(256), 0, st, ctx->d_part, ctx->d_bias[6], d_desc, n, npad, range_flag);
  ASD_HIP_CHECK(ctx, hipGetLastError());
  PROF_MARK(8);
#undef PROF_MARK
  if (prof) { ctx->prof_pending[pset] = true; ctx->prof_pending_n[pset] = n; ctx->prof_cur ^= 1; }
  return ASD_OK;
}

static int asdnet_calibrate(asd_ctx* ctx, const float* const conv_w[7], const float* const bn_mean[7], const float* const bn_var[7], float eps) {
  ctx->calib_note.clear();
  ctx->net_pieces = ctx->net_pieces_req;
  if (ctx->net_pieces != 2 || !(ctx->net_split & 31)) return ASD_OK;
  if (const char* e = getenv("ASD_ASDNET_CALIBRATE")) if (atoi(e) == 0) return ASD_OK;
  const int N = std::min(64, ctx->cfg.max_patches);
  constexpr float kCalibLimit = 2048.f;
  std::vector<uint8_t> pat((size_t)N * 1024);
  uint32_t rng = 0x9e3779b9u;
  auto rnd = [&]() { rng = rng * 1664525u + 1013904223u; return rng >> 8; };
  for (int p = 0; p < N; ++p)
    for (int y = 0; y < 32; ++y)
      for (int x = 0; x < 32; ++x) {
        int v;
        const int kind = p % 8, var = p / 8;
        switch (kind) {
          case 0: v = (int)(rnd() & 255); break;
          case 1: v = (x < 8 + 2 * var) ? 20 : 235; break;
          case 2: v = (y < 8 + 2 * var) ? 235 : 20; break;
          case 3: v = (x + y < 24 + 2 * var) ? 10 : 245; break;
          case 4: v = (((x >> (var % 3)) + (y >> (var % 3))) & 1) ? 255 : 0; break;
          case 5: v = (x * 255) / 31; break;
          case 6: v = (x == 4 * var + 1 && y == 3 * var + 2) ? 255 : 0; break;
          default: v = 128 + (int)(rnd() & 3); break;
        }
        pat[(size_t)p * 1024 + y * 32 + x] = (uint8_t)v;
      }
  float max1 = 0.f;
  {
    std::vector<float> inv(32), bias(32);
    for (int c = 0; c < 32; ++c) { inv[c] = 1.0f / std::sqrt(bn_var[0][c] + eps); bias[c] = -bn_mean[0][c] * inv[c]; }
    std::vector<float> in(34 * 34);
    for (int p = 0; p < N; ++p) {
      double s1 = 0, s2 = 0;
      for (int i = 0; i < 1024; ++i) s1 += pat[(size_t)p * 1024 + i] / 255.0;
      const double mean = s1 / 1024;
      for (int i = 0; i < 1024; ++i) { const double d = pat[(size_t)p * 1024 + i] / 255.0 - mean; s2 += d * d; }
      const double sd = std::sqrt(s2 / 1023) + 1e-7;
      std::fill(in.begin(), in.end(), 0.f);
      for (int y = 0; y < 32; ++y)
        for (int x = 0; x < 32; ++x) in[(y + 1) * 34 + x + 1] = (float)((pat[(size_t)p * 1024 + y * 32 + x] / 255.0 - mean) / sd);
      for (int c = 0; c < 32; ++c)
        for (int y = 0; y < 32; ++y)
          for (int x = 0; x < 32; ++x) {
            float a = bias[c];
            for (int k = 0; k < 9; ++k) a += in[(y + k / 3) * 34 + x + k % 3] * conv_w[0][c * 9 + k] * inv[c];
            max1 = std::max(max1, a);
          }
    }
  }
  uint8_t* d_pat = nullptr;
  unsigned* d_max = nullptr;
  float* d_out = nullptr;
  int rc = ASD_OK;
  unsigned hmax[8] = {};
  do {
    if (hipMalloc(&d_pat, pat.size()) != hipSuccess || hipMalloc(&d_max, 8 * sizeof(unsigned)) != hipSuccess ||
        hipMalloc(&d_out, (size_t)N * 128 * sizeof(float)) != hipSuccess) { rc = ASD_ERR_HIP; break; }
    if (hipMemcpy(d_pat, pat.data(), pat.size(), hipMemcpyHostToDevice) != hipSuccess || hipMemset(d_max, 0, 8 * sizeof(unsigned)) != hipSuccess) { rc = ASD_ERR_HIP; break; }
    ctx->d_calib = d_max;
    rc = asdnet_forward_device(ctx, d_pat, N, d_out, ctx->stream, nullptr);
    ctx->d_calib = nullptr;
    if (rc != ASD_OK) break;
    if (hipStreamSynchronize(ctx->stream) != hipSuccess || hipMemcpy(hmax, d_max, sizeof hmax, hipMemcpyDeviceToHost) != hipSuccess) rc = ASD_ERR_HIP;
  } while (0);
  if (d_pat) (void)hipFree(d_pat);
  if (d_max) (void)hipFree(d_max);
  if (d_out) (void)hipFree(d_out);
  if (rc != ASD_OK) { ctx->set_error("asd_load_weights: the range calibration pass failed"); return rc; }
  float worst = max1;
  int worst_layer = 1;
  for (int l = 1; l <= 5; ++l) {
    float v;
    memcpy(&v, &hmax[l], 4);
    if (!(v <= 3.0e38f)) v = INFINITY;
    if (v > worst) { worst = v; worst_layer = l + 1; }
  }
  if (worst > kCalibLimit) {
    ctx->net_pieces = 3;
    char buf[256];
    snprintf(buf, sizeof buf, "asd_load_weights: calibration found |activation| = %g behind conv%d (limit %g for the two-piece fp16 form): this context uses the three-piece bf16 form (asd_asdnet_pieces = 3)",
             (double)worst, worst_layer, (double)kCalibLimit);
    ctx->calib_note = buf;
  }
  return ASD_OK;
}

int asdnet_profile_collect_set(asd_ctx* ctx, int set) {
  if (!ctx->prof_pending[set]) return ASD_OK;
  ASD_HIP_CHECK(ctx, hipEventSynchronize(ctx->prof_ev[set][8]));
  for (int l = 0; l < 8; ++l) {
    float ms = 0;
    ASD_HIP_CHECK(ctx, hipEventElapsedTime(&ms, ctx->prof_ev[set][l], ctx->prof_ev[set][l + 1]));
    ctx->prof_ms[l] += ms;
    ctx->prof_calls[l] += 1;
    ctx->prof_patches[l] += ctx->prof_pending_n[set];
  }
  ctx->prof_pending[set] = false;
  return ASD_OK;
}

int asdnet_profile_collect(asd_ctx* ctx) {
  std::lock_guard<std::mutex> prof_lock(ctx->prof_mutex);
  for (int set = 0; set < 2; ++set) {
    const int rc = asdnet_profile_collect_set(ctx, set);
    if (rc != ASD_OK) return rc;
  }
  return ASD_OK;
}

template <int ABL>
static int ablate_one(asd_ctx* ctx, int layer, int n, int reps, float* ms) {
  hipStream_t st = ctx->stream;
  float *a0 = ctx->d_act[0], *a1 = ctx->d_act[1];
  hipError_t e = hipSuccess;
  auto run = [&](int count) {
    for (int r = 0; r < count; ++r) {
      if (layer == 2) {
        using C = ConvCfg<L2_CFG>;
        constexpr int rows = C::M_PATCH / C::HO;
        constexpr int lds = C::LDS_BYTES + ((rows + 4) * 36 + 320 + 8) * 4;
        auto k = k_conv_mfma<L2_CFG, ABL, true>;
        (void)hipFuncSetAttribute(reinterpret_cast<const void*>(k), hipFuncAttributeMaxDynamicSharedMemorySize, lds);
        hipLaunchKernelGGL(k, dim3(n * (C::HO / rows)), dim3(C::NTH), lds, st, (const void*)ctx->d_patches, ctx->d_wimg[1], ctx->d_bias[1], a1, ctx->d_w1, ctx->d_bias[0], n);
      } else if (layer == 4) {
        using C = ConvCfg<L4_CFG>;
        auto k = k_conv_mfma<L4_CFG, ABL, false>;
        (void)hipFuncSetAttribute(reinterpret_cast<const void*>(k), hipFuncAttributeMaxDynamicSharedMemorySize, C::LDS_BYTES);
        hipLaunchKernelGGL(k, dim3(n * (C::HO * C::HO / C::M_PATCH)), dim3(C::NTH), C::LDS_BYTES, st, (const void*)a0, ctx->d_wimg[3], ctx->d_bias[3], a1, (const float*)nullptr, (const float*)nullptr, n);
      } else {
        using C = ConvCfg<L6_CFG>;
        auto k = k_conv_mfma<L6_CFG, ABL, false>;
        (void)hipFuncSetAttribute(reinterpret_cast<const void*>(k), hipFuncAttributeMaxDynamicSharedMemorySize, C::LDS_BYTES);
        hipLaunchKernelGGL(k, dim3(((n + C::M_WG / C::M_PATCH - 1) / (C::M_WG / C::M_PATCH)) * (C::HO * C::HO / C::M_PATCH)), dim3(C::NTH), C::LDS_BYTES, st, (const void*)a0, ctx->d_wimg[5], ctx->d_bias[5], a1, (const float*)nullptr, (const float*)nullptr, n);
      }
    }
  };
  run(3);
  ASD_HIP_CHECK(ctx, hipEventRecord(ctx->ev0, st));
  run(reps);
  ASD_HIP_CHECK(ctx, hipEventRecord(ctx->ev1, st));
  ASD_HIP_CHECK(ctx, hipEventSynchronize(ctx->ev1));
  ASD_HIP_CHECK(ctx, hipEventElapsedTime(ms, ctx->ev0, ctx->ev1));
  *ms /= reps;
  (void)e;
  return ASD_OK;
}

extern "C" int asd_debug_act6(asd_ctx* ctx, int n, float* out) {
  if (n < 0 || n > ctx->cfg.max_patches) return ASD_ERR_CAPACITY;
  ASD_HIP_CHECK(ctx, hipStreamSynchronize(ctx->stream));
  const bool pair = kPairOK && ctx->net_pieces == 2 && (ctx->net_split & 63) == 63 && ctx->net_pair;
  const float* src = ctx->d_act6 ? ctx->d_act6 : ctx->d_act[1];
  if (!pair) { ASD_HIP_CHECK(ctx, hipMemcpy(out, src, (size_t)n * 8192 * 4, hipMemcpyDeviceToHost)); return ASD_OK; }
  std::vector<uint16_t> raw((size_t)n * 8192 * 2);
  ASD_HIP_CHECK(ctx, hipMemcpy(raw.data(), src, raw.size() * 2, hipMemcpyDeviceToHost));
  for (size_t e = 0; e < (size_t)n * 8192; ++e) {
    const size_t g = e / 8, j = e % 8;
    _Float16 h, l;
    memcpy(&h, &raw[g * 16 + j], 2);
    memcpy(&l, &raw[g * 16 + 8 + j], 2);
    out[e] = ((float)h + (float)l) / kActScale;
  }
  return ASD_OK;
}

extern "C" int asd_debug_x3_clock(asd_ctx* ctx, int layer, int n, int reps, double* loop_cycles, double* ghz) {
  hipStream_t st = ctx->stream;
  float *a0 = ctx->d_act[0], *a1 = ctx->d_act[1];
  unsigned long long* stamps = reinterpret_cast<unsigned long long*>(ctx->d_part);
  int grid = 0;
  for (int r = 0; r < reps; ++r) {
    unsigned long long* sp = r + 1 == reps ? stamps : nullptr;
    hipError_t e = hipErrorInvalidValue;
    const bool p2 = ctx->net_pieces == 2;
    const bool pair = kPairOK && p2 && (ctx->net_split & 63) == 63 && ctx->net_pair;
#define X3_CLK(CFG, FUSE, l, src, dst, w1p, b1p)                                                                                          \
  (pair ? launch_conv_x3<CFG, FUSE, 2, kPairOK>(st, src, ctx->d_wx2[l], ctx->d_bias[l], dst, n, w1p, b1p, sp, &grid, kActScale,               \
                                     1.f / (kActScale * ctx->wx2_scale[l]))                                                                \
   : p2 ? launch_conv_x3<CFG, FUSE, 2>(st, src, ctx->d_wx2[l], ctx->d_bias[l], dst, n, w1p, b1p, sp, &grid, kActScale,                       \
                                     1.f / (kActScale * ctx->wx2_scale[l]))                                                                \
      : launch_conv_x3<CFG, FUSE, 3>(st, src, ctx->d_wx3[l], ctx->d_bias[l], dst, n, w1p, b1p, sp, &grid))
    if (layer == 2) e = X3_CLK(L2S_CFG, true, 1, ctx->d_patches, a1, ctx->d_w1, ctx->d_bias[0]);
    else if (layer == 3) e = X3_CLK(L3S_CFG, false, 2, a1, a0, nullptr, nullptr);
    else if (layer == 4) e = X3_CLK(L4S_CFG, false, 3, a0, a1, nullptr, nullptr);
    else if (layer == 5) e = X3_CLK(L5S_CFG, false, 4, a1, a0, nullptr, nullptr);
    else if (layer == 6) e = X3_CLK(L6S_CFG, false, 5, a0, a1, nullptr, nullptr);
#undef X3_CLK
    ASD_HIP_CHECK(ctx, e);
  }
  ASD_HIP_CHECK(ctx, hipStreamSynchronize(st));
  if ((size_t)grid * 128 > (size_t)FC_SK * ((ctx->cfg.max_patches + 31) / 32 * 32) * 128 * sizeof(float)) return ASD_ERR_CAPACITY;
  std::vector<unsigned long long> hs((size_t)grid * 16);
  ASD_HIP_CHECK(ctx, hipMemcpy(hs.data(), stamps, hs.size() * 8, hipMemcpyDeviceToHost));
  std::vector<double> cyc(grid), rate(grid);
  for (int i = 0; i < grid; ++i) { cyc[i] = (double)hs[16 * i]; rate[i] = hs[16 * i + 1] ? (double)hs[16 * i] / (double)hs[16 * i + 1] : 0.0; }
  std::nth_element(cyc.begin(), cyc.begin() + grid / 2, cyc.end());
  std::nth_element(rate.begin(), rate.begin() + grid / 2, rate.end());
  *loop_cycles = cyc[grid / 2];
  *ghz = rate[grid / 2] * 0.1;
  if (getenv("ASD_X3_PHASES")) {
    auto med = [&](int k) { std::vector<double> v(grid); for (int i = 0; i < grid; ++i) v[i] = (double)hs[16 * i + k]; std::nth_element(v.begin(), v.begin() + grid / 2, v.end()); return v[grid / 2]; };
    fprintf(stderr, "  layer %d: %d workgroups; prologue %.0f, staging %.0f, MFMA loop %.0f, whole life %.0f cycles (medians)\n", layer, grid, med(2), med(3),
            med(0), med(5));
    if (layer == 2) fprintf(stderr, "     since entry: patch arrived %.0f, staging loop done %.0f, barrier passed %.0f\n", med(9), med(12), med(13));
  }
  return ASD_OK;
}

extern "C" int asd_debug_conv_ablate(asd_ctx* ctx, int layer, int n, int mode, int reps, float* ms) {
  switch (mode) {
    case 0: return ablate_one<0>(ctx, layer, n, reps, ms);
    case 1: return ablate_one<1>(ctx, layer, n, reps, ms);
    case 2: return ablate_one<2>(ctx, layer, n, reps, ms);
    case 3: return ablate_one<3>(ctx, layer, n, reps, ms);
    case 4: return ablate_one<4>(ctx, layer, n, reps, ms);
    case 5: return ablate_one<5>(ctx, layer, n, reps, ms);
    case 6: return ablate_one<6>(ctx, layer, n, reps, ms);
    case 7: return ablate_one<7>(ctx, layer, n, reps, ms);
    case 13: return ablate_one<13>(ctx, layer, n, reps, ms);
    case 21: return ablate_one<21>(ctx, layer, n, reps, ms);
    case 29: return ablate_one<29>(ctx, layer, n, reps, ms);
    default: return ASD_ERR_INVALID;
  }
}
```

asd-slam_amd/csrc/ctx.h:

```cpp
#pragma once
#include <hip/hip_runtime.h>

#include <atomic>
#include <cstdarg>
#include <cstdio>
#include <cstdlib>
#include <cstring>
#include <functional>
#include <mutex>
#include <string>
#include <vector>

#include "../../include/asd_slam.h"

#define ASD_HIP_CHECK(ctx, expr)                                                          \
  do {                                                                                    \
    hipError_t _e = (expr);                                                               \
    if (_e != hipSuccess) {                                                               \
      (ctx)->set_error("%s failed: %s (%s:%d)", #expr, hipGetErrorString(_e), __FILE__, __LINE__); \
      return ASD_ERR_HIP;                                                                 \
    }                                                                                     \
  } while (0)

struct AsdPerDeviceOnce {
  std::atomic<uint64_t> bits{0};
  bool need(int dev) const { return !((bits.load(std::memory_order_acquire) >> (dev & 63)) & 1); }
  void done(int dev) { bits.fetch_or(1ull << (dev & 63), std::memory_order_release); }
};

struct AsdDevBuf {
  void* p = nullptr;
  size_t cap = 0, used = 0;
  hipError_t reserve(size_t bytes) {
    used = 0;
    if (bytes <= cap) return hipSuccess;
    if (p) (void)hipFree(p);
    p = nullptr; cap = 0;
    const size_t want = bytes + bytes / 4 + 4096;
    const hipError_t e = hipMalloc(&p, want);
    if (e == hipSuccess) cap = want;
    return e;
  }
  template <typename T> T* carve(size_t count) {
    char* q = static_cast<char*>(p) + used;
    used += (count * sizeof(T) + 255) / 256 * 256;
    return reinterpret_cast<T*>(q);
  }
  static size_t padded(size_t bytes) { return (bytes + 255) / 256 * 256; }
  void release() { if (p) (void)hipFree(p); p = nullptr; cap = used = 0; }
};


hipError_t asd_copy_rows(hipStream_t st, void* dst, const void* src, size_t bytes);

#if defined(__HIPCC__)
#define asd_syncthreads() do { asm volatile("s_waitcnt lgkmcnt(0)" ::: "memory"); __syncthreads(); } while (0)
__device__ inline int asd_syncthreads_or(int pred) { asm volatile("s_waitcnt lgkmcnt(0)" ::: "memory"); return __syncthreads_or(pred); }
#endif


struct AsdWinQuery { float x, y, r; int min_level, max_level, qrow; };
struct AsdBetweenArgs {
  int n_cur, n_last, n_cand;
  const int* match1;
  const double* io1;
  const float* Xw_last;
  const int* last_cand;
  float T_pred[16];
  uint8_t* occ;
  float* cur_Xw;
  uint8_t* skip;
  float* T1;
};
#if defined(__HIPCC__)
template <class F>
__device__ inline void asd_frustum_bank_point(const F& a, const float* T_dev, const uint8_t* skip, const int q) {
#pragma clang fp contract(off)
  AsdWinQuery Q{0.f, 0.f, 0.f, 0, 0, -1};
  const int row = a.rows[q];
  const float4 A0 = reinterpret_cast<const float4*>(a.attr)[2 * (size_t)row], A1 = reinterpret_cast<const float4*>(a.attr)[2 * (size_t)row + 1];
  a.xw_out[3 * (size_t)q] = A0.x; a.xw_out[3 * (size_t)q + 1] = A0.y; a.xw_out[3 * (size_t)q + 2] = A0.z;
  if (!skip || !skip[q]) {
    float T[16], Ow[3];
    for (int i = 0; i < 16; ++i) T[i] = T_dev[i];
    for (int i = 0; i < 3; ++i) Ow[i] = T_dev[16 + i];
    const float P[3] = {A0.x, A0.y, A0.z}, Pn[3] = {A0.w, A1.x, A1.y};
    const float min_dist = A1.z, max_dist = A1.w;
    float Pc[3];
    for (int r = 0; r < 3; ++r) {
      const float t0 = T[r * 4 + 0] * P[0] + T[r * 4 + 1] * P[1] + T[r * 4 + 2] * P[2];
      Pc[r] = (float)((double)t0 + (double)T[r * 4 + 3]);
    }
    bool ok = !(Pc[2] < 0.0f);
    const float invz = 1.0f / Pc[2];
    const float u = a.fx * Pc[0] * invz + a.cx, v = a.fy * Pc[1] * invz + a.cy;
    if (u < a.min_x || u > a.max_x || v < a.min_y || v > a.max_y) ok = false;
    const float maxD = 1.2f * max_dist, minD = 0.8f * min_dist;
    const float PO[3] = {P[0] - Ow[0], P[1] - Ow[1], P[2] - Ow[2]};
    const double nn = (double)PO[0] * PO[0] + (double)PO[1] * PO[1] + (double)PO[2] * PO[2];
    const float dist = (float)sqrt(nn);
    if (dist < minD || dist > maxD) ok = false;
    const double dot = (double)PO[0] * Pn[0] + (double)PO[1] * Pn[1] + (double)PO[2] * Pn[2];
    const float vc = (float)(dot / dist);
    if (vc < a.cos_limit) ok = false;
    if (ok) {
      const float ratio = max_dist / dist;
      int lvl = 0;
      for (int k = 1; k < a.n_levels; ++k) lvl += ratio >= a.level_thr[k];
      float r = vc > 0.998 ? 2.5f : 4.0f;
      if (a.bfactor) r *= a.th;
      Q = AsdWinQuery{u, v, r * a.scale[lvl], lvl - 1, lvl, row};
    }
  }
  a.queries[q] = Q;
}
__device__ inline void asd_between_body(const AsdBetweenArgs& a_dev, const int t, const int nt) {
#pragma clang fp contract(off)
  const AsdBetweenArgs a = a_dev;
  __shared__ int s_nmatch;
  if (t == 0) s_nmatch = 0;
  for (int c = t; c < a.n_cand; c += nt) a.skip[c] = 0;
  asd_syncthreads();
  const uint8_t* outl = reinterpret_cast<const uint8_t*>(a.io1 + 8);
  int mine = 0;
  for (int j = t; j < a.n_cur; j += nt) {
    const int i = a.match1[j];
    mine += i >= 0;
    const int src = i >= 0 ? i : 0;
    for (int k = 0; k < 3; ++k) a.cur_Xw[3 * (size_t)j + k] = a.n_last > 0 ? a.Xw_last[3 * (size_t)src + k] : 0.f;
    const bool keep = i >= 0 && !outl[j];
    a.occ[j] = keep ? 1 : 0;
    if (i >= 0 && a.last_cand) { const int c = a.last_cand[i]; if (c >= 0 && c < a.n_cand) a.skip[c] = 1; }
  }
  if (mine) atomicAdd(&s_nmatch, mine);
  asd_syncthreads();
  if (t == 0) {
    float T[16];
    if (s_nmatch >= 3) {
      const double* p = a.io1;
      const double x = p[0], y = p[1], z = p[2], w = p[3];
      const double tx = 2 * x, ty = 2 * y, tz = 2 * z;
      const double twx = tx * w, twy = ty * w, twz = tz * w, txx = tx * x, txy = ty * x, txz = tz * x, tyy = ty * y, tyz = tz * y, tzz = tz * z;
      const double R[9] = {1 - (tyy + tzz), txy - twz, txz + twy, txy + twz, 1 - (txx + tzz), tyz - twx, txz - twy, tyz + twx, 1 - (txx + tyy)};
      for (int i = 0; i < 3; ++i) {
        for (int j = 0; j < 3; ++j) T[i * 4 + j] = (float)R[i * 3 + j];
        T[i * 4 + 3] = (float)p[4 + i];
      }
      T[12] = T[13] = T[14] = 0.f;
      T[15] = 1.f;
    } else {
      for (int i = 0; i < 16; ++i) T[i] = a.T_pred[i];
    }
    for (int i = 0; i < 16; ++i) a.T1[i] = T[i];
    for (int i = 0; i < 3; ++i) {
      double sum = 0;
      for (int k = 0; k < 3; ++k) sum += (double)T[k * 4 + i] * (double)T[k * 4 + 3];
      a.T1[16 + i] = (float)(-1.0 * sum);
    }
  }
}
#endif

struct AsdXfer {
  char* h = nullptr;
  char* d = nullptr;
  size_t cap = 0, used = 0;
  hipError_t begin(hipStream_t st, size_t bytes) {
    used = 0;
    bytes += 4096;
    if (bytes <= cap) return hipSuccess;
    if (h) { (void)hipStreamSynchronize(st); (void)hipHostFree(h); (void)hipFree(d); }
    h = nullptr; d = nullptr; cap = 0;
    const size_t want = bytes + bytes / 2;
    hipError_t e = hipHostMalloc(&h, want);
    if (e == hipSuccess) e = hipMalloc(&d, want);
    if (e == hipSuccess) cap = want;
    return e;
  }
  size_t reserve(size_t bytes) { const size_t off = used; used += (bytes + 255) / 256 * 256; return off; }
  size_t add(const void* src, size_t bytes) { const size_t off = reserve(bytes); memcpy(h + off, src, bytes); return off; }
  size_t zeros(size_t bytes) { const size_t off = reserve(bytes); memset(h + off, 0, bytes); return off; }
  hipError_t upload(hipStream_t st) {
    if (!used) return hipSuccess;
    static const bool by_kernel = getenv("ASD_UPLOAD_COPY") == nullptr;
    return by_kernel ? asd_copy_rows(st, d, h, (used + 15) / 16 * 16) : hipMemcpyAsync(d, h, used, hipMemcpyHostToDevice, st);
  }
  hipError_t download(hipStream_t st) { return used ? hipMemcpyAsync(h, d, used, hipMemcpyDeviceToHost, st) : hipSuccess; }
  template <typename T> T* dev(size_t off) { return reinterpret_cast<T*>(d + off); }
  template <typename T> T* host(size_t off) { return reinterpret_cast<T*>(h + off); }
  void release() { if (h) (void)hipHostFree(h); if (d) (void)hipFree(d); h = d = nullptr; cap = used = 0; }
};

struct AsdFrameSlot {
  int n = 0;
  float min_x = 0, max_x = 0, min_y = 0, max_y = 0;
  float inv_w = 0, inv_h = 0;
  std::vector<asd_keypoint> kps;
  std::vector<int32_t> cell_start;
  std::vector<int32_t> cell_items;
  float* d_desc = nullptr;
  float4* d_kp = nullptr;
  int32_t* d_cell_start = nullptr;
  int32_t* d_cell_items = nullptr;
  int32_t* d_fv = nullptr;
  int32_t fv_nodes = 0;
  char* h_stage = nullptr;
  hipEvent_t ev_staged = nullptr;
};

struct UndistortMap {
  int w = 0, h = 0, mpitch = 0;
  short2* d_xy = nullptr;
  uint16_t* d_frac = nullptr;
  uint8_t* d_io = nullptr;
};

struct asd_ctx {
  asd_config cfg{};
  hipStream_t stream = nullptr;
  hipStream_t stream_x = nullptr;
  hipStream_t stream_prep = nullptr;
  hipEvent_t ev_prep = nullptr;
  bool prep_on = false;
  struct AsyncExtract* ax = nullptr;
  int num_cu = 256;
  std::string err;

  float scale[ASD_MAX_LEVELS], inv_scale[ASD_MAX_LEVELS], sigma2[ASD_MAX_LEVELS], inv_sigma2[ASD_MAX_LEVELS];
  int features_per_level[ASD_MAX_LEVELS];
  float level_thr[ASD_MAX_LEVELS];
  int umax[16];

  bool weights_loaded = false;
  float* d_w1 = nullptr;
  float* d_bias[7] = {};
  float* d_wimg[7] = {};
  void* d_wx3[7] = {};
  bool match_replay_host = false;
  bool ba_struct_host = false;
  void* d_wx2[7] = {};
  float wx2_scale[7] = {1, 1, 1, 1, 1, 1, 1};
  int net_pieces_req = 2;
  int net_pieces = 2;
  int net_split = 1;
  float* d_act[2] = {};
  float* d_part = nullptr;
  int* h_range = nullptr;
  std::string calib_note;
  unsigned* d_calib = nullptr;
  bool pose_chain_kp_flags = false;
  bool net_pair = true;
  float* d_act6 = nullptr;
  int ring_mask = 0;
  uint8_t* d_patches = nullptr;
  float* d_desc = nullptr;
  bool keep_pyramid = false;
  const uint8_t* d_pyr_view = nullptr;
  AsdDevBuf stereo_scratch;
  float* d_desc_last = nullptr;
  hipEvent_t ev_adopt = nullptr;
  bool adopt_pending = false;

  struct FrontendState* fe = nullptr;
  UndistortMap* und = nullptr;
  int last_n = 0;

  AsdFrameSlot frames[ASD_MAX_FRAMES];

  void* matcher = nullptr;

  void* ba = nullptr;

  AsdDevBuf scratch;
  AsdXfer up, down;
  bool track_async_armed = false, track_has_pending = false;
  hipEvent_t ev_chain = nullptr;
  std::function<int()> track_pending;

  void* mapping = nullptr;

  void* bow = nullptr;

  std::mutex prof_mutex;
  bool prof_on = false;
  hipEvent_t prof_ev[2][9] = {};
  bool prof_pending[2] = {false, false};
  int prof_pending_n[2] = {0, 0};
  int prof_cur = 0;
  double prof_ms[8] = {};
  int prof_calls[8] = {};
  long long prof_patches[8] = {};

  hipEvent_t ev0 = nullptr, ev1 = nullptr, ev2 = nullptr;
  float ms_asdnet = 0, ms_extract = 0, ms_match = 0, ms_ba = 0;

  std::mutex err_mutex;
  std::string err_returned;
  void set_error(const char* fmt, ...) {
    char buf[512];
    va_list ap;
    va_start(ap, fmt);
    vsnprintf(buf, sizeof buf, fmt, ap);
    va_end(ap);
    std::lock_guard<std::mutex> l(err_mutex);
    err = buf;
  }
  const char* last_error() {
    std::lock_guard<std::mutex> l(err_mutex);
    err_returned = err;
    return err_returned.c_str();
  }
};

inline hipStream_t asd_prep_stream(asd_ctx* ctx) { return ctx->prep_on ? ctx->stream_prep : ctx->stream; }

int frontend_alloc(asd_ctx* ctx);
void frontend_free(asd_ctx* ctx);
void frontend_async_shutdown(asd_ctx* ctx);
bool asd_extractor_busy(asd_ctx* ctx, const char* who);
int frontend_image_to_device(asd_ctx* ctx, const uint8_t* image, bool on_device, int width, int height, int stride, uint8_t* dst,
                             int pitch, hipStream_t st);
int undistort_launch(asd_ctx* ctx, const UndistortMap& U, hipStream_t st, const uint8_t* src, int stride, uint8_t* dst, int pitch);
void undistort_free(asd_ctx* ctx);
bool asd_track_busy(asd_ctx* ctx, const char* who);
void matcher_free(asd_ctx* ctx);
void ba_free(asd_ctx* ctx);
void mapping_free(asd_ctx* ctx);
void bow_free(asd_ctx* ctx);
struct AsdFusedReplay { const void* args; int kind; int nq; size_t lds; };
bool pose_chain_fused_ok(const asd_ctx* ctx, int kind, int nq, int n_cur, size_t lds);
int pose_chain_enqueue(asd_ctx* ctx, int n_cur, const int* d_src, const float4* d_kp, const float* d_tab, const uint8_t* d_hold,
                       const float* d_own, const double* pose7, const double* K, double* d_io, const double* d_pose0 = nullptr,
                       double* d_io_dev = nullptr, const AsdBetweenArgs* between = nullptr, const AsdFusedReplay* fused = nullptr);
int pose_chain_reserve(asd_ctx* ctx, int n_cur);
inline bool pose_chain_lds_form(const asd_ctx* ctx, int n_cur) { return ctx->cfg.n_levels <= 16 && (size_t)n_cur * 35 + 16 <= 150 * 1024; }
inline size_t pose_chain_io_bytes(int n_cur) { return 64 + ((size_t)n_cur + 7) / 8 * 8 + 64; }
void asd_compute_quotas(int nfeatures, float scaleFactor, int nl, int* out);

inline int asd_range_status(asd_ctx* ctx, int* flag, const char* who) {
  if (!flag || !*flag) return ASD_OK;
  *flag = 0;
  ctx->set_error("%s: an ASDNet activation left the range of the two-piece fp16 operand form (|x| > 4094): the descriptors of this call are "
                 "not valid.  ASD_ASDNET_MATH=bf16x3 (or f32) has no range limit", who);
  return ASD_ERR_RANGE;
}
int asdnet_alloc(asd_ctx* ctx);
void asdnet_free(asd_ctx* ctx);
int asdnet_load_weights(asd_ctx* ctx, const float* const conv_w[7], const float* const bn_mean[7],
                        const float* const bn_var[7], float eps);
int asdnet_forward_device(asd_ctx* ctx, const uint8_t* d_patches, int n, float* d_desc, hipStream_t st, int* range_flag = nullptr);
int asdnet_profile_collect(asd_ctx* ctx);
int asdnet_ring_conv(asd_ctx* ctx, int layer, const void* in, void* out, int n, hipStream_t st);
int asdnet_ring_conv45(asd_ctx* ctx, const void* in, void* out, int n, hipStream_t st);
```

Measured before the change: 1250.

## Fuse conv2 and conv3 into one kernel keeping conv2 output in LDS

Adds a kernel that runs conv1+conv2 and then conv3 in the same workgroup. The conv2 result is written as packed f16 pair pieces straight into LDS and consumed there by the stride-2 conv3 MFMA loop, so it no longer round-trips through a global activation buffer and one launch is saved. Shared helpers (tile pixel mapping, B loads, MFMA loop, pair store, conv1 fill) are factored out so both paths can use them. The path is on by default when the pair format is active, with an environment switch to turn it off. In exchange the kernel needs more LDS per workgroup, which can lower occupancy.

Result: no change. 1267, median of 4 (+1.3%).

```diff
diff --git a/asd-slam_amd/csrc/asdnet.hip b/asd-slam_amd/csrc/asdnet.hip
--- a/asd-slam_amd/csrc/asdnet.hip
+++ b/asd-slam_amd/csrc/asdnet.hip
@@ -419,7 +419,9 @@
   static constexpr int NC16 = CIN / KCH;
   static constexpr int NCHUNK = 9 * NC16;
   static constexpr int CHUNKB = KCH * 2 * NP * COUT;
-  static constexpr int ACT_BYTES = INROWS * INCOLS * PIXB;
+  static constexpr int NPIX = INROWS * INCOLS;
+  static constexpr int NCOUT = COUT;
+  static constexpr int ACT_BYTES = NPIX * PIXB;
   static constexpr int LDS_BYTES = PP * ACT_BYTES;
   static_assert((PIXB / 16) % 2 == 1, "pixel stride must be an odd multiple of 16 B");
   static constexpr int NCW = COUT / WN;
@@ -499,6 +501,249 @@
   asd_syncthreads();
   const float sd = sqrtf(((red[4] + red[5]) + (red[6] + red[7])) * (1.0f / 1023.0f)) + 1e-7f;
   if (t == 0) { stats[2 * (size_t)patch] = mean; stats[2 * (size_t)patch + 1] = sd; }
+}
+
+template <int S, int HO, int NP, int PP, int ROWS>
+__device__ __forceinline__ int x3_tile_pixel(int sg, int r16) {
+  if constexpr (NP == 2 && ASD_X3_S16) {
+    if constexpr (S == 1 && HO >= 16) return sg * 16 + (r16 < 4 ? 2 * r16 : r16 < 12 ? 2 * r16 - 7 : 2 * r16 - 16);
+    else if constexpr (S == 2 && HO >= 16) return sg * 16 + r16;
+    else if constexpr (S == 2) return sg * 16 + (r16 < 4 ? r16 : r16 < 12 ? r16 + 4 : r16 - 8);
+    else {
+      static_assert(S == 2 || HO >= 16 || (PP == 1 && HO == 8 && ROWS == 8), "eight rows x two columns per sub-tile");
+      const int j = r16 < 4 ? r16 : r16 < 12 ? r16 - 4 : r16 - 8;
+      return j * HO + 2 * sg + (r16 >= 4 && r16 < 12 ? 1 : 0);
+    }
+  } else return sg * (ASD_X3_S16 ? 16 : 32) + r16;
+}
+
+template <class G, int S, int PP, int ROWS, int NP, int NA>
+__device__ __forceinline__ void x3_abase(int sg0, int lr, int kg, int (&abase)[NA]) {
+  for (int ma = 0; ma < NA; ++ma) {
+    const int m = x3_tile_pixel<S, G::HO, NP, PP, ROWS>(sg0 + ma, lr);
+    const int pp = PP > 1 ? m / G::M_PATCH : 0, mm = m - pp * G::M_PATCH;
+    const int rr = mm / G::HO, ox = mm % G::HO;
+    abase[ma] = pp * G::ACT_BYTES + ((rr * S) * G::INCOLS + ox * S) * G::PIXB + kg * G::GSTR;
+  }
+}
+
+template <class G, int NP, int NB>
+__device__ __forceinline__ void x3_load_b(const uint8_t* wl, int c, u32x4 (&b)[NB][NP]) {
+  constexpr int KG = G::KCH / 8, TW = ASD_X3_S16 ? 16 : 32;
+  const uint8_t* wc = wl + (size_t)((ASD_X3_ABL & 1) ? (c & 1) : c) * G::CHUNKB;
+#pragma unroll
+  for (int nb = 0; nb < NB; ++nb)
+#pragma unroll
+    for (int p = 0; p < NP; ++p) b[nb][p] = *reinterpret_cast<const u32x4*>(wc + (size_t)p * KG * G::NCOUT * 16 + nb * TW * 16);
+}
+
+template <int NP, bool PAIR, class ACC>
+__device__ __forceinline__ void x3_mma(const u32x4& x, const u32x4& y, ACC& c) {
+  auto bf = [](const u32x4& v) { return __builtin_bit_cast(bf16x8, v); };
+  auto hf = [](const u32x4& v) { return __builtin_bit_cast(f16x8, v); };
+  constexpr bool S16 = ASD_X3_S16;
+  if constexpr ((ASD_X3_ABL & 8) != 0) { asm volatile("" ::"v"(x), "v"(y)); }
+#ifdef ASD_PAIR_NOTRANS
+  else if constexpr (PAIR) c = __builtin_amdgcn_mfma_f32_16x16x32_f16(hf(x), hf(y), c, 0, 0, 0);
+#endif
+  else if constexpr (PAIR) c = __builtin_amdgcn_mfma_f32_16x16x32_f16(hf(y), hf(x), c, 0, 0, 0);
+  else if constexpr (NP == 2 && S16) c = __builtin_amdgcn_mfma_f32_16x16x32_f16(hf(x), hf(y), c, 0, 0, 0);
+  else if constexpr (NP == 2) c = __builtin_amdgcn_mfma_f32_32x32x16_f16(hf(x), hf(y), c, 0, 0, 0);
+  else if constexpr (S16) c = __builtin_amdgcn_mfma_f32_16x16x32_bf16(bf(x), bf(y), c, 0, 0, 0);
+  else c = __builtin_amdgcn_mfma_f32_32x32x16_bf16(bf(x), bf(y), c, 0, 0, 0);
+}
+
+template <class G, int NP, bool PAIR, int NA, int NB, int RB, class ACC, class F>
+__device__ __forceinline__ void x3_mfma_loop(const uint8_t* wl, u32x4 (&br)[RB][NB][NP], const int (&abase)[NA], ACC (&acc)[NA][NB], F at_start) {
+  extern __shared__ __attribute__((aligned(16))) uint8_t smem_b[];
+  constexpr int KG = G::KCH / 8;
+  static_assert(G::NCHUNK % RB == 0, "chunk count");
+  auto chunk_off = [&](int c) {
+    const int tap = c / G::NC16, c16 = c % G::NC16;
+    return ((tap / 3) * G::INCOLS + (tap % 3)) * G::PIXB + c16 * (KG * G::GSTR);
+  };
+  auto load_a = [&](int off, u32x4 (&a)[NP]) {
+#pragma unroll
+    for (int p = 0; p < NP; ++p) a[p] = *reinterpret_cast<const u32x4*>(smem_b + off + p * G::PSTR);
+  };
+  constexpr int PD = ASD_X3_PD, RS = PD + 1;
+  static_assert((RB * NA) % RS == 0, "ring slots must be static");
+  u32x4 ar[RS][NP];
+#pragma unroll
+  for (int q = 0; q < PD; ++q) load_a(abase[q % NA] + chunk_off(q / NA), ar[q]);
+  at_start();
+  for (int c0 = 0; c0 < G::NCHUNK; c0 += RB) {
+    int offs[RB + PD / NA + 2];
+#pragma unroll
+    for (int u = 0; u < RB + PD / NA + 2; ++u) offs[u] = chunk_off(c0 + u < G::NCHUNK ? c0 + u : G::NCHUNK - 1);
+#pragma unroll
+    for (int u = 0; u < RB; ++u) {
+      const int c = c0 + u;
+      x3_load_b<G, NP, NB>(wl, c + RB - 1 < G::NCHUNK ? c + RB - 1 : G::NCHUNK - 1, br[(u + RB - 1) % RB]);
+      __builtin_amdgcn_sched_group_barrier(0x020, NP * NB, 0);
+      const u32x4 (&bc)[NB][NP] = br[u];
+#pragma unroll
+      for (int ma = 0; ma < NA; ++ma) {
+        const int q = u * NA + ma;
+        const int qn = q + PD;
+        load_a(abase[qn % NA] + offs[qn / NA], ar[qn % RS]);
+        const u32x4 (&ac)[NP] = ar[q % RS];
+#pragma unroll
+        for (int nb = 0; nb < NB; ++nb) {
+          if constexpr (NP == 2) {
+            x3_mma<NP, PAIR>(ac[1], bc[nb][0], acc[ma][nb]);
+            x3_mma<NP, PAIR>(ac[0], bc[nb][1], acc[ma][nb]);
+            x3_mma<NP, PAIR>(ac[0], bc[nb][0], acc[ma][nb]);
+          } else {
+            x3_mma<NP, PAIR>(ac[2], bc[nb][0], acc[ma][nb]);
+            x3_mma<NP, PAIR>(ac[0], bc[nb][2], acc[ma][nb]);
+            x3_mma<NP, PAIR>(ac[1], bc[nb][1], acc[ma][nb]);
+            x3_mma<NP, PAIR>(ac[1], bc[nb][0], acc[ma][nb]);
+            x3_mma<NP, PAIR>(ac[0], bc[nb][1], acc[ma][nb]);
+            x3_mma<NP, PAIR>(ac[0], bc[nb][0], acc[ma][nb]);
+          }
+        }
+#pragma unroll
+        for (int p = 0; p < NP; ++p) {
+          __builtin_amdgcn_sched_group_barrier(0x008, (NP * (NP + 1) / 2) * NB / NP, 0);
+          __builtin_amdgcn_sched_group_barrier(0x100, 1, 0);
+        }
+      }
+    }
+  }
+}
+
+template <class ACC>
+__device__ __forceinline__ u32x4 x3_pair_pieces(const ACC& a, const f32x4& bv, float out_scale, uint32_t& probe) {
+  float v[4];
+#pragma unroll
+  for (int r = 0; r < 4; ++r) { const float x = a[r] * out_scale + bv[r]; v[r] = x < 0.f ? 0.f : x; }
+  uint32_t hh[2], ll[2];
+  split4_mix(v[0], v[1], v[2], v[3], kActScale, hh, ll);
+  const auto s0 = __builtin_amdgcn_permlane16_swap(hh[0], ll[0], false, false);
+  const auto s1 = __builtin_amdgcn_permlane16_swap(hh[1], ll[1], false, false);
+  probe = hh[0];
+  return u32x4{s0[0], s1[0], s0[1], s1[1]};
+}
+
+template <class C, int COUT, int S, int ROWS, int PP, int NA, int NB, class ACC>
+__device__ __forceinline__ void x3_pair_store(float* out, const float* bias, const ACC (&acc)[NA][NB], int patch, int r0,
+                                              int sg0, int co_w, int kg, int lr, int n, float out_scale) {
+  constexpr int TW = 16;
+  uint8_t* opb = reinterpret_cast<uint8_t*>(out) + ((size_t)patch * C::HO + r0) * C::HO * COUT * 4;
+  for (int nb = 0; nb < NB; ++nb) {
+    const int co0 = co_w + nb * TW + 4 * kg;
+    const f32x4 bv = *reinterpret_cast<const f32x4*>(bias + co0);
+    for (int ma = 0; ma < NA; ++ma) {
+      const int m0 = (sg0 + ma) * TW;
+      const int pp = PP > 1 ? m0 / C::M_PATCH : 0;
+      if (PP > 1 && patch + pp >= n) continue;
+      const int m = x3_tile_pixel<S, C::HO, 2, PP, ROWS>(sg0 + ma, lr);
+      uint32_t probe;
+      const u32x4 pc = x3_pair_pieces(acc[ma][nb], bv, out_scale, probe);
+      uint8_t* o = opb + ((size_t)pp * C::HO * C::HO + (size_t)(m - pp * C::M_PATCH)) * COUT * 4 + (co0 >> 3) * 32 + (kg & 1) * 16;
+      if (!(ASD_X3_ABL & 4) || probe == 0x12345u) *reinterpret_cast<u32x4*>(o) = pc;
+    }
+  }
+}
+
+template <class G, int ROWS, int NP, int NW, bool SCRATCH, class Pin, class Stamp>
+__device__ __forceinline__ void x3_conv1_fill(Pin pin, float* wsh, float* red, const uint8_t* patches,
+                                              const float* w1, const float* b1, const float* stats,
+                                              int patch, int r0, float in_scale, int t, Stamp stamp, unsigned long long& st_t1, bool stamps) {
+  extern __shared__ __attribute__((aligned(16))) uint8_t smem_b[];
+  constexpr int NTH = 64 * NW;
+  const int lane = t & 63, wave = t >> 6;
+  const int q = t & 3;
+  float wq[8][9], bq1[8];
+  auto load_wq = [&](const float* wsrc, const float* bsrc) {
+#pragma unroll
+    for (int c = 0; c < 8; ++c) {
+      bq1[c] = bsrc[8 * q + c];
+#pragma unroll
+      for (int k = 0; k < 9; ++k) wq[c][k] = wsrc[(8 * q + c) * 9 + k];
+    }
+  };
+  if constexpr (!SCRATCH) load_wq(w1, b1);
+  for (int i = t; i < (ROWS + 4) * 36; i += NTH) {
+    const int j = i / 36, c = i % 36, y = r0 - 2 + j;
+    if (!(c >= 1 && c <= 32 && y >= 0 && y < 32)) pin(i) = 0.f;
+  }
+  if constexpr (SCRATCH) {
+    for (int i = t; i < 288; i += NTH) wsh[i] = w1[i];
+    if (t < 32) wsh[288 + t] = b1[t];
+  }
+  const bool ld = NW == 4 || wave < 4;
+  const uchar4 v = ld ? reinterpret_cast<const uchar4*>(patches + (size_t)patch * 1024)[t] : make_uchar4(0, 0, 0, 0);
+  const float inv255 = (float)(1.0 / 255);
+  float x[4] = {v.x * inv255, v.y * inv255, v.z * inv255, v.w * inv255};
+#pragma unroll
+  for (int k = 0; k < 4; ++k) asm volatile("" : "+v"(x[k]));
+  float d[4], sd;
+  if (!SCRATCH || stats) {
+    const float mean = stats[2 * (size_t)patch];
+    sd = stats[2 * (size_t)patch + 1];
+    for (int k = 0; k < 4; ++k) d[k] = x[k] - mean;
+    stamp(9);
+  } else {
+    float sum = (x[0] + x[1]) + (x[2] + x[3]);
+    for (int off = 32; off >= 1; off >>= 1) sum += __shfl_xor(sum, off);
+    stamp(9);
+    if (lane == 0 && ld) red[wave] = sum;
+    asd_syncthreads();
+    const float mean = ((red[0] + red[1]) + (red[2] + red[3])) * (1.0f / 1024.0f);
+    float ss = 0.f;
+    for (int k = 0; k < 4; ++k) { d[k] = x[k] - mean; ss += d[k] * d[k]; }
+    for (int off = 32; off >= 1; off >>= 1) ss += __shfl_xor(ss, off);
+    if (lane == 0 && ld) red[4 + wave] = ss;
+    asd_syncthreads();
+    sd = sqrtf(((red[4] + red[5]) + (red[6] + red[7])) * (1.0f / 1023.0f)) + 1e-7f;
+  }
+  if (ld) {
+    const int idx = t * 4, y = idx >> 5, x0 = idx & 31;
+    const int j = y - (r0 - 2);
+    if (j >= 0 && j < ROWS + 4)
+      for (int k = 0; k < 4; ++k) pin(j * 36 + x0 + k + 1) = d[k] / sd;
+  }
+  asd_syncthreads();
+  if (stamps) st_t1 = __builtin_amdgcn_s_memtime();
+  if (!(ASD_X3_ABL & 2)) {
+    if constexpr (SCRATCH) load_wq(wsh, wsh + 288);
+    for (int item = t; item < G::NPIX * 4; item += NTH) {
+      const int pix = item >> 2;
+      const int i = pix % G::INCOLS, j = pix / G::INCOLS;
+      const int oy = r0 - 1 + j, ox = i - 1;
+      f32x4 ra = {0.f, 0.f, 0.f, 0.f}, rb = {0.f, 0.f, 0.f, 0.f};
+      if (oy >= 0 && oy < 32 && ox >= 0 && ox < 32) {
+        float a[9];
+#pragma unroll
+        for (int ky = 0; ky < 3; ++ky)
+#pragma unroll
+          for (int kx = 0; kx < 3; ++kx) a[ky * 3 + kx] = pin((j + ky) * 36 + ox + kx);
+#pragma unroll
+        for (int c = 0; c < 8; ++c) {
+          float acc1 = bq1[c];
+#pragma unroll
+          for (int k = 0; k < ((ASD_X3_ABL & 32) ? 1 : 9); ++k) acc1 += a[k] * wq[c][k];
+          const float r = acc1 > 0.f ? acc1 : 0.f;
+          if (c < 4) ra[c] = r; else rb[c - 4] = r;
+        }
+      }
+      u32x4 ph, pm, pl;
+      uint8_t* dst = smem_b + pix * G::PIXB + q * G::GSTR;
+      if constexpr (NP == 2) {
+        split8_f16(ra, rb, in_scale, ph, pl);
+        *reinterpret_cast<u32x4*>(dst) = ph;
+        *reinterpret_cast<u32x4*>(dst + G::PSTR) = pl;
+      } else {
+        if constexpr ((ASD_X3_ABL & 64) != 0) { ph = __builtin_bit_cast(u32x4, ra); pm = __builtin_bit_cast(u32x4, rb); pl = ph; }
+        else split8(ra, rb, ph, pm, pl);
+        *reinterpret_cast<u32x4*>(dst) = ph;
+        *reinterpret_cast<u32x4*>(dst + 16) = pm;
+        *reinterpret_cast<u32x4*>(dst + 32) = pl;
+      }
+    }
+  }
 }
 
 template <int CIN, int COUT, int HIN, int S, int ROWS, int WM, int WN, int PP, bool FUSE1 = false, int NP = 3, bool PAIR = false>
@@ -524,114 +769,22 @@
 #define X3_STAMP(k) do { if (stamps && t == 0) stamps[16 * bid + (k)] = __builtin_amdgcn_s_memtime() - st_t0; } while (0)
 
   constexpr bool S16 = ASD_X3_S16;
-  constexpr int SUB = S16 ? 2 : 1, KG = C::KCH / 8, TW = 32 / SUB;
+  constexpr int SUB = S16 ? 2 : 1, TW = 32 / SUB;
   const int kg = S16 ? lane >> 4 : h, lr = S16 ? lane & 15 : li;
   const uint8_t* wl = wimg + ((size_t)kg * COUT + wn * NCW + lr) * 16;
   constexpr int NB = NCW / TW;
-  auto load_b = [&](int c, u32x4 (&b)[NB][NP]) {
-    const uint8_t* wc = wl + (size_t)((ASD_X3_ABL & 1) ? (c & 1) : c) * C::CHUNKB;
-#pragma unroll
-    for (int nb = 0; nb < NB; ++nb)
-#pragma unroll
-      for (int p = 0; p < NP; ++p) b[nb][p] = *reinterpret_cast<const u32x4*>(wc + (size_t)p * KG * COUT * 16 + nb * TW * 16);
-  };
   constexpr int RB = C::NCHUNK % ASD_X3_RB == 0 ? ASD_X3_RB : 3;
-  static_assert(C::NCHUNK % RB == 0, "chunk count");
   u32x4 br[RB][NB][NP];
 #pragma unroll
-  for (int d = 0; d < RB - 1; ++d) load_b(d, br[d]);
+  for (int d = 0; d < RB - 1; ++d) x3_load_b<C, NP, NB>(wl, d, br[d]);
 
   if constexpr (FUSE1) {
     static_assert(!FUSE1 || (CIN == 32 && HIN == 32 && S == 1 && PP == 1 && (C::NW == 4 || C::NW == 8)), "conv1 fusion is for conv2 only");
     float* pin = reinterpret_cast<float*>(smem_b + C::ACT_BYTES);
     float* wsh = pin + (ROWS + 4) * 36;
     float* red = wsh + 320;
-    const uint8_t* patches = static_cast<const uint8_t*>(in_);
-    for (int i = t; i < (ROWS + 4) * 36; i += NTH) {
-      const int j = i / 36, c = i % 36, y = r0 - 2 + j;
-      if (!(c >= 1 && c <= 32 && y >= 0 && y < 32)) pin[i] = 0.f;
-    }
-    for (int i = t; i < 288; i += NTH) wsh[i] = w1[i];
-    if (t < 32) wsh[288 + t] = b1[t];
-    const bool ld = C::NW == 4 || wave < 4;
-    const uchar4 v = ld ? reinterpret_cast<const uchar4*>(patches + (size_t)patch * 1024)[t] : make_uchar4(0, 0, 0, 0);
-    const float inv255 = (float)(1.0 / 255);
-    float x[4] = {v.x * inv255, v.y * inv255, v.z * inv255, v.w * inv255};
-#pragma unroll
-    for (int k = 0; k < 4; ++k) asm volatile("" : "+v"(x[k]));
-    float d[4], sd;
-    if (stats) {
-      const float mean = stats[2 * (size_t)patch];
-      sd = stats[2 * (size_t)patch + 1];
-      for (int k = 0; k < 4; ++k) d[k] = x[k] - mean;
-      X3_STAMP(9);
-    } else {
-      float sum = (x[0] + x[1]) + (x[2] + x[3]);
-      for (int off = 32; off >= 1; off >>= 1) sum += __shfl_xor(sum, off);
-      X3_STAMP(9);
-      if (lane == 0 && ld) red[wave] = sum;
-      asd_syncthreads();
-      const float mean = ((red[0] + red[1]) + (red[2] + red[3])) * (1.0f / 1024.0f);
-      float ss = 0.f;
-      for (int k = 0; k < 4; ++k) { d[k] = x[k] - mean; ss += d[k] * d[k]; }
-      for (int off = 32; off >= 1; off >>= 1) ss += __shfl_xor(ss, off);
-      if (lane == 0 && ld) red[4 + wave] = ss;
-      asd_syncthreads();
-      sd = sqrtf(((red[4] + red[5]) + (red[6] + red[7])) * (1.0f / 1023.0f)) + 1e-7f;
-    }
-    if (ld) {
-      const int idx = t * 4, y = idx >> 5, x0 = idx & 31;
-      const int j = y - (r0 - 2);
-      if (j >= 0 && j < ROWS + 4)
-        for (int k = 0; k < 4; ++k) pin[j * 36 + x0 + k + 1] = d[k] / sd;
-    }
-    asd_syncthreads();
-    if (stamps) st_t1 = __builtin_amdgcn_s_memtime();
-    constexpr int NPIX = C::INROWS * C::INCOLS;
-    if (!(ASD_X3_ABL & 2)) {
-      const int q = t & 3;
-      float wq[8][9], bq1[8];
-#pragma unroll
-      for (int c = 0; c < 8; ++c) {
-        bq1[c] = wsh[288 + 8 * q + c];
-#pragma unroll
-        for (int k = 0; k < 9; ++k) wq[c][k] = wsh[(8 * q + c) * 9 + k];
-      }
-      for (int item = t; item < NPIX * 4; item += NTH) {
-        const int pix = item >> 2;
-        const int i = pix % C::INCOLS, j = pix / C::INCOLS;
-        const int oy = r0 - 1 + j, ox = i - 1;
-        f32x4 ra = {0.f, 0.f, 0.f, 0.f}, rb = {0.f, 0.f, 0.f, 0.f};
-        if (oy >= 0 && oy < 32 && ox >= 0 && ox < 32) {
-          float a[9];
-#pragma unroll
-          for (int ky = 0; ky < 3; ++ky)
-#pragma unroll
-            for (int kx = 0; kx < 3; ++kx) a[ky * 3 + kx] = pin[(j + ky) * 36 + ox + kx];
-#pragma unroll
-          for (int c = 0; c < 8; ++c) {
-            float acc1 = bq1[c];
-#pragma unroll
-            for (int k = 0; k < ((ASD_X3_ABL & 32) ? 1 : 9); ++k) acc1 += a[k] * wq[c][k];
-            const float r = acc1 > 0.f ? acc1 : 0.f;
-            if (c < 4) ra[c] = r; else rb[c - 4] = r;
-          }
-        }
-        u32x4 ph, pm, pl;
-        uint8_t* dst = smem_b + pix * C::PIXB + q * C::GSTR;
-        if constexpr (NP == 2) {
-          split8_f16(ra, rb, in_scale, ph, pl);
-          *reinterpret_cast<u32x4*>(dst) = ph;
-          *reinterpret_cast<u32x4*>(dst + C::PSTR) = pl;
-        } else {
-          if constexpr ((ASD_X3_ABL & 64) != 0) { ph = __builtin_bit_cast(u32x4, ra); pm = __builtin_bit_cast(u32x4, rb); pl = ph; }
-          else split8(ra, rb, ph, pm, pl);
-          *reinterpret_cast<u32x4*>(dst) = ph;
-          *reinterpret_cast<u32x4*>(dst + 16) = pm;
-          *reinterpret_cast<u32x4*>(dst + 32) = pl;
-        }
-      }
-    }
+    x3_conv1_fill<C, ROWS, NP, C::NW, true>([&](int i) -> float& { return pin[i]; }, wsh, red, static_cast<const uint8_t*>(in_), w1, b1,
+                                            stats, patch, r0, in_scale, t, [&](int k) { X3_STAMP(k); }, st_t1, stamps != nullptr);
   } else if constexpr (PAIR) {
     const uint8_t* inb = static_cast<const uint8_t*>(in_) + (size_t)patch * HIN * HIN * CIN * 4;
     constexpr int C8 = CIN / 8;
@@ -721,93 +874,12 @@
   for (int ma = 0; ma < NA; ++ma)
     for (int nb = 0; nb < NB; ++nb)
       for (int r = 0; r < AR; ++r) acc[ma][nb][r] = 0.f;
-  auto tile_pixel = [&](int sg, int r16) -> int {
-    if constexpr (NP == 2 && S16) {
-      if constexpr (S == 1 && C::HO >= 16) return sg * 16 + (r16 < 4 ? 2 * r16 : r16 < 12 ? 2 * r16 - 7 : 2 * r16 - 16);
-      else if constexpr (S == 2 && C::HO >= 16) return sg * 16 + r16;
-      else if constexpr (S == 2) return sg * 16 + (r16 < 4 ? r16 : r16 < 12 ? r16 + 4 : r16 - 8);
-      else {
-        static_assert(S == 2 || C::HO >= 16 || (PP == 1 && C::HO == 8 && ROWS == 8), "eight rows x two columns per sub-tile");
-        const int j = r16 < 4 ? r16 : r16 < 12 ? r16 - 4 : r16 - 8;
-        return j * C::HO + 2 * sg + (r16 >= 4 && r16 < 12 ? 1 : 0);
-      }
-    } else return sg * TW + r16;
-  };
+  auto tile_pixel = [&](int sg, int r16) -> int { return x3_tile_pixel<S, C::HO, NP, PP, ROWS>(sg, r16); };
   int abase[NA];
-  for (int ma = 0; ma < NA; ++ma) {
-    const int m = tile_pixel((wm * MT * 32 + ma * TW) / TW, lr);
-    const int pp = PP > 1 ? m / C::M_PATCH : 0, mm = m - pp * C::M_PATCH;
-    const int rr = mm / C::HO, ox = mm % C::HO;
-    abase[ma] = pp * C::ACT_BYTES + ((rr * S) * C::INCOLS + ox * S) * C::PIXB + kg * C::GSTR;
-  }
-  auto chunk_off = [&](int c) {
-    const int tap = c / C::NC16, c16 = c % C::NC16;
-    return ((tap / 3) * C::INCOLS + (tap % 3)) * C::PIXB + c16 * (KG * C::GSTR);
-  };
-  auto load_a = [&](int off, u32x4 (&a)[NP]) {
-#pragma unroll
-    for (int p = 0; p < NP; ++p) a[p] = *reinterpret_cast<const u32x4*>(smem_b + off + p * C::PSTR);
-  };
-  auto bf = [](const u32x4& v) { return __builtin_bit_cast(bf16x8, v); };
-  auto hf = [](const u32x4& v) { return __builtin_bit_cast(f16x8, v); };
-  auto mma = [&](const u32x4& x, const u32x4& y, accv& c) {
-    if constexpr ((ASD_X3_ABL & 8) != 0) { asm volatile("" ::"v"(x), "v"(y)); }
-#ifdef ASD_PAIR_NOTRANS
-    else if constexpr (PAIR) c = __builtin_amdgcn_mfma_f32_16x16x32_f16(hf(x), hf(y), c, 0, 0, 0);
-#endif
-    else if constexpr (PAIR) c = __builtin_amdgcn_mfma_f32_16x16x32_f16(hf(y), hf(x), c, 0, 0, 0);
-    else if constexpr (NP == 2 && S16) c = __builtin_amdgcn_mfma_f32_16x16x32_f16(hf(x), hf(y), c, 0, 0, 0);
-    else if constexpr (NP == 2) c = __builtin_amdgcn_mfma_f32_32x32x16_f16(hf(x), hf(y), c, 0, 0, 0);
-    else if constexpr (S16) c = __builtin_amdgcn_mfma_f32_16x16x32_bf16(bf(x), bf(y), c, 0, 0, 0);
-    else c = __builtin_amdgcn_mfma_f32_32x32x16_bf16(bf(x), bf(y), c, 0, 0, 0);
-  };
-
-  constexpr int PD = ASD_X3_PD, RS = PD + 1;
-  static_assert((RB * NA) % RS == 0, "ring slots must be static");
-  u32x4 ar[RS][NP];
-#pragma unroll
-  for (int q = 0; q < PD; ++q) load_a(abase[q % NA] + chunk_off(q / NA), ar[q]);
+  x3_abase<C, S, PP, ROWS, NP, NA>(wm * NA, lr, kg, abase);
   unsigned long long st_c = 0, st_r = 0;
-  if (stamps) { st_c = __builtin_amdgcn_s_memtime(); st_r = __builtin_amdgcn_s_memrealtime(); }
-  for (int c0 = 0; c0 < C::NCHUNK; c0 += RB) {
-    int offs[RB + PD / NA + 2];
-#pragma unroll
-    for (int u = 0; u < RB + PD / NA + 2; ++u) offs[u] = chunk_off(c0 + u < C::NCHUNK ? c0 + u : C::NCHUNK - 1);
-#pragma unroll
-    for (int u = 0; u < RB; ++u) {
-      const int c = c0 + u;
-      load_b(c + RB - 1 < C::NCHUNK ? c + RB - 1 : C::NCHUNK - 1, br[(u + RB - 1) % RB]);
-      __builtin_amdgcn_sched_group_barrier(0x020, NP * NB, 0);
-      const u32x4 (&bc)[NB][NP] = br[u];
-#pragma unroll
-      for (int ma = 0; ma < NA; ++ma) {
-        const int q = u * NA + ma;
-        const int qn = q + PD;
-        load_a(abase[qn % NA] + offs[qn / NA], ar[qn % RS]);
-        const u32x4 (&ac)[NP] = ar[q % RS];
-#pragma unroll
-        for (int nb = 0; nb < NB; ++nb) {
-          if constexpr (NP == 2) {
-            mma(ac[1], bc[nb][0], acc[ma][nb]);
-            mma(ac[0], bc[nb][1], acc[ma][nb]);
-            mma(ac[0], bc[nb][0], acc[ma][nb]);
-          } else {
-            mma(ac[2], bc[nb][0], acc[ma][nb]);
-            mma(ac[0], bc[nb][2], acc[ma][nb]);
-            mma(ac[1], bc[nb][1], acc[ma][nb]);
-            mma(ac[1], bc[nb][0], acc[ma][nb]);
-            mma(ac[0], bc[nb][1], acc[ma][nb]);
-            mma(ac[0], bc[nb][0], acc[ma][nb]);
-          }
-        }
-#pragma unroll
-        for (int p = 0; p < NP; ++p) {
-          __builtin_amdgcn_sched_group_barrier(0x008, (NP * (NP + 1) / 2) * NB / NP, 0);
-          __builtin_amdgcn_sched_group_barrier(0x100, 1, 0);
-        }
-      }
-    }
-  }
+  x3_mfma_loop<C, NP, PAIR, NA, NB, RB>(wl, br, abase, acc,
+                                        [&]() { if (stamps) { st_c = __builtin_amdgcn_s_memtime(); st_r = __builtin_amdgcn_s_memrealtime(); } });
 
   if (stamps) {
     asm volatile("s_nop 0" ::"v"(acc[NA - 1][NB - 1][0]));
@@ -824,15 +896,10 @@
         const int pp = PP > 1 ? m0 / C::M_PATCH : 0;
         if (PP > 1 && patch + pp >= n) continue;
         const int m = tile_pixel(m0 / TW, lr);
-        float v[4];
-#pragma unroll
-        for (int r = 0; r < 4; ++r) { const float x = acc[ma][nb][r] * out_scale + bv[r]; v[r] = x < 0.f ? 0.f : x; }
-        uint32_t hh[2], ll[2];
-        split4_mix(v[0], v[1], v[2], v[3], kActScale, hh, ll);
-        const auto s0 = __builtin_amdgcn_permlane16_swap(hh[0], ll[0], false, false);
-        const auto s1 = __builtin_amdgcn_permlane16_swap(hh[1], ll[1], false, false);
+        uint32_t probe;
+        const u32x4 pc = x3_pair_pieces(acc[ma][nb], bv, out_scale, probe);
         uint8_t* o = opb + ((size_t)pp * C::HO * C::HO + (size_t)(m - pp * C::M_PATCH)) * COUT * 4 + (co0 >> 3) * 32 + (kg & 1) * 16;
-        if (!(ASD_X3_ABL & 4) || hh[0] == 0x12345u) *reinterpret_cast<u32x4*>(o) = u32x4{s0[0], s1[0], s0[1], s1[1]};
+        if (!(ASD_X3_ABL & 4) || probe == 0x12345u) *reinterpret_cast<u32x4*>(o) = pc;
       }
     }
   } else {
@@ -1155,6 +1222,104 @@
 #define L5S_CFG 64, 128, 16, 2, ASD_L5_RWMN, 1
 #define L6S_CFG 128, 128, 8, 1, 8, ASD_L6_WMN, 1
 
+#if ASD_X3_S16
+struct X3L23A {
+  using L2 = X3Cfg<32, 32, 32, 1, 8, 4, 1, 1, 2>;
+  static constexpr int ROWS = 9, HO = 32, INROWS = ROWS + 2, INCOLS = 33;
+  static constexpr int NPIX = INROWS * INCOLS + 1;
+  static constexpr int PIXB = L2::PIXB, GSTR = L2::GSTR, PSTR = L2::PSTR, KCH = L2::KCH, NC16 = L2::NC16, NCHUNK = L2::NCHUNK;
+  static constexpr int CHUNKB = L2::CHUNKB, NCOUT = 32, M_PATCH = ROWS * HO, ACT_BYTES = NPIX * PIXB;
+  static constexpr int WM = 2, WN = 2, NA = 9, NB = 1;
+  static_assert(WM * NA * 16 == M_PATCH && WN * NB * 16 == NCOUT, "wave split");
+  static_assert(((ROWS + 4) * 36 + 3) / 4 <= NPIX && PIXB - 16 == 32 * 2 * 2, "the normalised input rows fit the pixel pads");
+};
+using X3L23B = X3Cfg<L3S_CFG, 2>;
+constexpr int kL23LdsBytes = X3L23A::ACT_BYTES > X3L23B::ACT_BYTES ? X3L23A::ACT_BYTES : X3L23B::ACT_BYTES;
+constexpr int kLdsGranule = 1280;
+static_assert(X3L23B::INROWS == X3L23A::ROWS && X3L23B::INCOLS == 33 && X3L23B::MT == 2 && X3L23B::NCW == 16 && X3L23B::NW == 4 && X3L23B::PLANAR,
+              "the fused kernel is written for conv3 as four rows per band, 1 x 4 waves");
+static_assert(kL23LdsBytes <= 54613 && (kL23LdsBytes + kLdsGranule - 1) / kLdsGranule * 3 <= 160 * 1024 / kLdsGranule,
+              "conv2 + conv3: three workgroups per CU");
+
+__global__ __launch_bounds__(256, 3) void k_conv_x3_l23(const uint8_t* __restrict__ patches, const uint8_t* __restrict__ w2img, const float* __restrict__ bias2,
+                                                        const uint8_t* __restrict__ w3img, const float* __restrict__ bias3, float* __restrict__ out,
+                                                        const float* __restrict__ w1, const float* __restrict__ b1, int n,
+                                                        unsigned long long* __restrict__ stamps, float out_scale2, float out_scale3,
+                                                        const float* __restrict__ stats) {
+  using A = X3L23A;
+  using B = X3L23B;
+  extern __shared__ __attribute__((aligned(16))) uint8_t smem_b[];
+  const int bid = blockIdx.x;
+  int t = threadIdx.x;
+  asm volatile("" : "+v"(t));
+  const int lane = t & 63, wave = t >> 6, kg = lane >> 4, lr = lane & 15;
+  const int patch = bid >> 2, band = bid & 3;
+  const int r0 = 8 * band - 1;
+  unsigned long long st_t0 = 0, st_t1 = 0, st_c = 0, st_r = 0, st_e = 0, st_c3 = 0;
+  if (stamps) st_t0 = st_t1 = __builtin_amdgcn_s_memtime();
+  auto stamp = [&](int k) { if (stamps && t == 0) stamps[16 * bid + k] = __builtin_amdgcn_s_memtime() - st_t0; };
+  typedef float accv __attribute__((ext_vector_type(4)));
+  constexpr int RB = 3;
+
+  const int wm2 = wave / A::WN, wn2 = wave % A::WN;
+  const uint8_t* wl2 = w2img + ((size_t)kg * A::NCOUT + wn2 * 16 + lr) * 16;
+  u32x4 br2[RB][A::NB][2];
+#pragma unroll
+  for (int d = 0; d < RB - 1; ++d) x3_load_b<A, 2, A::NB>(wl2, d, br2[d]);
+  x3_conv1_fill<A, A::ROWS, 2, 4, false>([&](int i) -> float& { return *reinterpret_cast<float*>(smem_b + (i >> 2) * A::PIXB + (A::PIXB - 16) + (i & 3) * 4); },
+                                        nullptr, nullptr, patches, w1, b1, stats, patch, r0, kActScale, t, stamp, st_t1, stamps != nullptr);
+  stamp(12);
+  asd_syncthreads();
+  stamp(13);
+
+  accv acc2[A::NA][A::NB];
+  for (int ma = 0; ma < A::NA; ++ma)
+    for (int r = 0; r < 4; ++r) acc2[ma][0][r] = 0.f;
+  int abase2[A::NA];
+  x3_abase<A, 1, 1, A::ROWS, 2, A::NA>(wm2 * A::NA, lr, kg, abase2);
+  x3_mfma_loop<A, 2, true, A::NA, A::NB, RB>(wl2, br2, abase2, acc2,
+                                             [&]() { if (stamps) { st_c = __builtin_amdgcn_s_memtime(); st_r = __builtin_amdgcn_s_memrealtime(); } });
+  if (stamps) {
+    asm volatile("s_nop 0" ::"v"(acc2[A::NA - 1][0][0]));
+    st_e = __builtin_amdgcn_s_memtime();
+    const unsigned long long e_r = __builtin_amdgcn_s_memrealtime();
+    if (t == 0) { stamps[16 * bid] = st_e - st_c; stamps[16 * bid + 1] = e_r - st_r; stamps[16 * bid + 2] = st_t1 - st_t0; stamps[16 * bid + 3] = st_c - st_t1; stamps[16 * bid + 6] = st_t0; }
+  }
+  const uint8_t* wl3 = w3img + ((size_t)kg * B::NCOUT + wave * B::NCW + lr) * 16;
+  u32x4 br3[RB][1][2];
+#pragma unroll
+  for (int d = 0; d < RB - 1; ++d) x3_load_b<B, 2, 1>(wl3, d, br3[d]);
+  asd_syncthreads();
+  {
+    const int co0 = wn2 * 16 + 4 * kg;
+    const f32x4 bv = *reinterpret_cast<const f32x4*>(bias2 + co0);
+    for (int ma = 0; ma < A::NA; ++ma) {
+      const int m = x3_tile_pixel<1, A::HO, 2, 1, A::ROWS>(wm2 * A::NA + ma, lr);
+      const int rr = m / A::HO, ox = m % A::HO;
+      uint32_t probe;
+      u32x4 pc = x3_pair_pieces(acc2[ma][0], bv, out_scale2, probe);
+      if (band == 0 && rr == 0) pc = u32x4{0, 0, 0, 0};
+      *reinterpret_cast<u32x4*>(smem_b + (rr * B::INCOLS + ox + 1) * B::PIXB + (co0 >> 3) * B::GSTR + (kg & 1) * B::PSTR) = pc;
+    }
+    if (t < A::ROWS * 8) *reinterpret_cast<u32x4*>(smem_b + (t >> 3) * B::INCOLS * B::PIXB + (t & 7) * 16) = u32x4{0, 0, 0, 0};
+  }
+  asd_syncthreads();
+  accv acc3[4][1];
+  for (int ma = 0; ma < 4; ++ma)
+    for (int r = 0; r < 4; ++r) acc3[ma][0][r] = 0.f;
+  int abase3[4];
+  x3_abase<B, 2, 1, ASD_L3_ROWS, 2, 4>(0, lr, kg, abase3);
+  x3_mfma_loop<B, 2, true, 4, 1, RB>(wl3, br3, abase3, acc3, [&]() { if (stamps) st_c3 = __builtin_amdgcn_s_memtime(); });
+  if (stamps) {
+    asm volatile("s_nop 0" ::"v"(acc3[3][0][0]));
+    const unsigned long long e = __builtin_amdgcn_s_memtime();
+    if (t == 0) { stamps[16 * bid + 8] = st_c3 - st_e; stamps[16 * bid + 10] = e - st_c3; }
+  }
+  x3_pair_store<B, 64, 2, ASD_L3_ROWS, 1>(out, bias3, acc3, patch, band * ASD_L3_ROWS, 0, wave * B::NCW, kg, lr, n, out_scale3);
+  if (stamps && t == 0) { const unsigned long long e = __builtin_amdgcn_s_memtime(); stamps[16 * bid + 5] = e - st_t0; stamps[16 * bid + 7] = e; }
+}
+#endif
+
 template <int CIN, int COUT, int HIN, int S, int ROWS, int WM, int WN, int KC, int PP = 1, int RING = 2, bool FUSE1 = false>
 hipError_t launch_conv(hipStream_t st, const void* in, const float* wimg, const float* bias, float* out, int n,
                        const float* w1 = nullptr, const float* b1 = nullptr) {
@@ -1219,6 +1384,25 @@
   return hipGetLastError();
 }
 
+#if ASD_X3_S16
+hipError_t launch_conv_x3_l23(hipStream_t st, const uint8_t* patches, const void* w2img, const float* bias2, const void* w3img, const float* bias3, float* out,
+                              int n, const float* w1, const float* b1, float out_scale2, float out_scale3, const float* stats,
+                              unsigned long long* stamps = nullptr, int* grid_out = nullptr) {
+  static AsdPerDeviceOnce attr_set;
+  int dev_ = 0;
+  (void)hipGetDevice(&dev_);
+  if (attr_set.need(dev_)) {
+    hipError_t e = hipFuncSetAttribute(reinterpret_cast<const void*>(k_conv_x3_l23), hipFuncAttributeMaxDynamicSharedMemorySize, kL23LdsBytes);
+    if (e != hipSuccess) return e;
+    attr_set.done(dev_);
+  }
+  if (grid_out) *grid_out = 4 * n;
+  hipLaunchKernelGGL(k_conv_x3_l23, dim3(4 * n), dim3(256), kL23LdsBytes, st, patches, static_cast<const uint8_t*>(w2img), bias2,
+                     static_cast<const uint8_t*>(w3img), bias3, out, w1, b1, n, stamps, out_scale2, out_scale3, stats);
+  return hipGetLastError();
+}
+#endif
+
 inline void split3_host(float x, uint16_t& h, uint16_t& m, uint16_t& l) {
   uint32_t u, r1u, r2u;
   memcpy(&u, &x, 4);
@@ -1291,6 +1475,7 @@
   *ctx->h_range = 0;
   if (const char* e = getenv("ASD_ASDNET_PAIR")) ctx->net_pair = atoi(e) != 0;
   if (const char* e = getenv("ASD_ASDNET_RING")) ctx->ring_mask = atoi(e);
+  if (const char* e = getenv("ASD_ASDNET_FUSE23")) ctx->net_fuse23 = atoi(e) != 0;
   return ASD_OK;
 }
 
@@ -1408,6 +1593,7 @@
   PROF_MARK(1);
   const bool p2 = ctx->net_pieces == 2;
   const bool pair = kPairOK && p2 && (ctx->net_split & 63) == 63 && ctx->net_pair && !ctx->d_calib;
+  const bool fuse23 = ASD_X3_S16 && pair && ctx->net_fuse23;
   const float* x3_stats = nullptr;
 #define X3_LAUNCH(CFG, FUSE, l, src, dst, w1p, b1p)                                                                                       \
   (pair ? launch_conv_x3<CFG, FUSE, 2, kPairOK>(st, src, ctx->d_wx2[l], ctx->d_bias[l], dst, n, w1p, b1p, nullptr, nullptr, kActScale,       \
@@ -1420,6 +1606,12 @@
     hipLaunchKernelGGL(k_patch_stats, dim3(n), dim3(256), 0, st, d_patches, ctx->d_part, n);
     ASD_HIP_CHECK(ctx, hipGetLastError());
     x3_stats = ctx->d_part;
+#if ASD_X3_S16
+    if (fuse23)
+      ASD_HIP_CHECK(ctx, launch_conv_x3_l23(st, d_patches, ctx->d_wx2[1], ctx->d_bias[1], ctx->d_wx2[2], ctx->d_bias[2], a0, n, ctx->d_w1, ctx->d_bias[0],
+                                            1.f / (kActScale * ctx->wx2_scale[1]), 1.f / (kActScale * ctx->wx2_scale[2]), x3_stats));
+    else
+#endif
     ASD_HIP_CHECK(ctx, (X3_LAUNCH(L2S_CFG, true, 1, d_patches, a1, ctx->d_w1, ctx->d_bias[0])));
     x3_stats = nullptr;
   }
@@ -1427,7 +1619,8 @@
 #define CALIB(l, buf, elems) do { if (ctx->d_calib) { hipLaunchKernelGGL(k_absmax, dim3(256), dim3(256), 0, st, buf, (size_t)n * (elems), ctx->d_calib + (l)); ASD_HIP_CHECK(ctx, hipGetLastError()); } } while (0)
   CALIB(1, a1, 32 * 32 * 32);
   PROF_MARK(2);
-  if (ctx->net_split & 2) ASD_HIP_CHECK(ctx, (X3_LAUNCH(L3S_CFG, false, 2, a1, a0, nullptr, nullptr)));
+  if (fuse23) {}
+  else if (ctx->net_split & 2) ASD_HIP_CHECK(ctx, (X3_LAUNCH(L3S_CFG, false, 2, a1, a0, nullptr, nullptr)));
   else
   ASD_HIP_CHECK(ctx, (launch_conv_p<L3_CFG>(st, a1, ctx->d_wimg[2], ctx->d_bias[2], a0, n, ctx->num_cu)));
   CALIB(2, a0, 16 * 16 * 64);
@@ -1642,11 +1835,19 @@
   return ASD_OK;
 }
 
+extern "C" int asd_debug_fuse23(asd_ctx* ctx) {
+  return ASD_X3_S16 && kPairOK && ctx->net_pieces == 2 && (ctx->net_split & 63) == 63 && ctx->net_pair && ctx->net_fuse23;
+}
+
 extern "C" int asd_debug_x3_clock(asd_ctx* ctx, int layer, int n, int reps, double* loop_cycles, double* ghz) {
   hipStream_t st = ctx->stream;
   float *a0 = ctx->d_act[0], *a1 = ctx->d_act[1];
   unsigned long long* stamps = reinterpret_cast<unsigned long long*>(ctx->d_part);
   int grid = 0;
+  if (layer == 23) {
+    hipLaunchKernelGGL(k_patch_stats, dim3(n), dim3(256), 0, st, ctx->d_patches, ctx->d_part + 16 * 4 * 2 * (size_t)n, n);
+    ASD_HIP_CHECK(ctx, hipGetLastError());
+  }
   for (int r = 0; r < reps; ++r) {
     unsigned long long* sp = r + 1 == reps ? stamps : nullptr;
     hipError_t e = hipErrorInvalidValue;
@@ -1663,6 +1864,11 @@
     else if (layer == 4) e = X3_CLK(L4S_CFG, false, 3, a0, a1, nullptr, nullptr);
     else if (layer == 5) e = X3_CLK(L5S_CFG, false, 4, a1, a0, nullptr, nullptr);
     else if (layer == 6) e = X3_CLK(L6S_CFG, false, 5, a0, a1, nullptr, nullptr);
+#if ASD_X3_S16
+    else if (layer == 23 && pair)
+      e = launch_conv_x3_l23(st, ctx->d_patches, ctx->d_wx2[1], ctx->d_bias[1], ctx->d_wx2[2], ctx->d_bias[2], a0, n, ctx->d_w1, ctx->d_bias[0],
+                             1.f / (kActScale * ctx->wx2_scale[1]), 1.f / (kActScale * ctx->wx2_scale[2]), ctx->d_part + 16 * 4 * 2 * (size_t)n, sp, &grid);
+#endif
 #undef X3_CLK
     ASD_HIP_CHECK(ctx, e);
   }
@@ -1680,7 +1886,15 @@
     auto med = [&](int k) { std::vector<double> v(grid); for (int i = 0; i < grid; ++i) v[i] = (double)hs[16 * i + k]; std::nth_element(v.begin(), v.begin() + grid / 2, v.end()); return v[grid / 2]; };
     fprintf(stderr, "  layer %d: %d workgroups; prologue %.0f, staging %.0f, MFMA loop %.0f, whole life %.0f cycles (medians)\n", layer, grid, med(2), med(3),
             med(0), med(5));
-    if (layer == 2) fprintf(stderr, "     since entry: patch arrived %.0f, staging loop done %.0f, barrier passed %.0f\n", med(9), med(12), med(13));
+#if ASD_X3_S16
+    if (layer == 23) {
+      int per_cu = 0;
+      (void)hipOccupancyMaxActiveBlocksPerMultiprocessor(&per_cu, reinterpret_cast<const void*>(k_conv_x3_l23), 256, kL23LdsBytes);
+      fprintf(stderr, "     conv2 + conv3: MFMA loop above = conv2's; LDS epilogue %.0f, conv3 loop %.0f cycles; %d B of LDS, %d workgroups per CU (hipOccupancyMaxActiveBlocksPerMultiprocessor)\n",
+              med(8), med(10), kL23LdsBytes, per_cu);
+    }
+#endif
+    if (layer == 2 || layer == 23) fprintf(stderr, "     since entry: patch arrived %.0f, staging loop done %.0f, barrier passed %.0f\n", med(9), med(12), med(13));
   }
   return ASD_OK;
 }
diff --git a/asd-slam_amd/csrc/ctx.h b/asd-slam_amd/csrc/ctx.h
--- a/asd-slam_amd/csrc/ctx.h
+++ b/asd-slam_amd/csrc/ctx.h
@@ -250,6 +250,7 @@
   unsigned* d_calib = nullptr;
   bool pose_chain_kp_flags = false;
   bool net_pair = true;
+  bool net_fuse23 = true;
   float* d_act6 = nullptr;
   int ring_mask = 0;
   uint8_t* d_patches = nullptr;
```
